# opteroncx/MoePhoto

Hardware: AMD Instinct MI355X
Metric: megapixels/sec (input), 1080p 4x SR (Net4x a4), 256-px tiles with overlap (higher is better)
Workload: dtype fp16; 1 GPU; BASELINE configs[1]: 1 frame(s) 1920x1080 RGB -> 7680x4320, model a4 (Net4x, synthetic weights in zoo format), crop 256 pad 5 align 8 -> 40 tiles/frame, fp16 I/O, fp16 MFMA operands + fp32 accumulate; tiles_per_frame=40, parallelism=single GPU, precision=mixed, exact_blocks=1, input=natural-image-like synthetic frame (tests/golden_defs.natural_image)

## Files before the change

### include/moephoto_amd.h

```cpp
#ifndef MOEPHOTO_AMD_H
#define MOEPHOTO_AMD_H

#include <stddef.h>
#include <stdint.h>

#ifdef __cplusplus
extern "C" {
#endif

#define MOE_ABI_VERSION 4

#define MOE_OK 0
#define MOE_EINVAL (-1)
#define MOE_ENOMEM (-2)
#define MOE_EHIP (-3)
#define MOE_ESTATE (-4)

#define MOE_ARCH_NET2X 0
#define MOE_ARCH_NET3X 1
#define MOE_ARCH_NET4X 2
#define MOE_ARCH_NETDN 3
#define MOE_ARCH_SEDN 4
#define MOE_ARCH_LITE 5

// ... 2 lines not shown
#define MOE_U8 2
#define MOE_U16 3

#define MOE_PREC_FP16 0
#define MOE_PREC_FP16X3 1
#define MOE_PREC_DEBUG_DIRECT 2
#define MOE_PREC_MIXED 3

#define MOE_PREC_AUTO 4

typedef struct moe_net moe_net;
typedef struct moe_plan moe_plan;

const char* moe_last_error(void);
int moe_abi_version(void);
int moe_device_count(void);

int moe_device_info(int device, int64_t info[8]);

int moe_net_create(int arch, int scale, moe_net** out);
void moe_net_destroy(moe_net* net);
int moe_net_scale(const moe_net* net);
int moe_net_num_params(const moe_net* net);
int moe_net_param_info(const moe_net* net, int index, const char** name, int64_t shape[4], int* ndim);
int moe_net_set_param(moe_net* net, const char* name, const float* data, const int64_t* shape, int ndim);
int moe_net_finalize(moe_net* net, int device, int precision);
int moe_net_resolved_precision(const moe_net* net, int precision);
int moe_net_calibrate(moe_net* net, double target, int* blocks, double* err, void* stream);
int moe_net_exact_blocks(const moe_net* net);
int64_t moe_net_workspace_bytes(const moe_net* net, int B, int h, int w);
int64_t moe_net_max_tile_pixels(const moe_net* net);
int moe_net_forward(moe_net* net, const void* x, int x_dtype, int B, int h, int w,
                    int64_t sB, int64_t sH, int64_t sW, const int64_t* x_off,
                    void* y, int y_dtype, const int64_t* y_off, void* stream);
#define MOE_FWD_INPUT_SINCE_PREV 1u
int moe_net_forward_ex(moe_net* net, const void* x, int x_dtype, int B, int h, int w,
                       int64_t sB, int64_t sH, int64_t sW, const int64_t* x_off,
                       void* y, int y_dtype, const int64_t* y_off, void* stream, unsigned flags);
int moe_net_set_profile(moe_net* net, const char* layer_substrings);
int moe_net_get_profile_at(moe_net* net, int index, double* total_ms, int64_t* launches, double* flops);
int moe_net_get_profile(moe_net* net, double* total_ms, int64_t* launches, double* flops);
int moe_net_set_exact_blocks(moe_net* net, int blocks);
int moe_net_set_option(moe_net* net, const char* key, const char* value);
int moe_net_set_debug(moe_net* net, int enable);
int64_t moe_net_debug_tap(moe_net* net, const char* tap, float* host, int64_t capacity, int64_t shape[4], void* stream);

int moe_plan_create(const int64_t shape[3], double ram, double ram_coef, int pad, int scale, int align,
                    int cropsize, moe_plan** out);
void moe_plan_destroy(moe_plan* plan);
int moe_plan_info(const moe_plan* plan, int64_t info[12]);
int moe_plan_tiles(const moe_plan* plan, int32_t* tiles);
int moe_plan_ramp(const moe_plan* plan, float* ramp);
int moe_plan_rows(const moe_plan* plan, int32_t* rows);

int moe_stitch(const moe_plan* plan, int device, const float* tiles_dev, const int64_t* tile_off, int C,
               void* out, int out_dtype, void* stream);
int moe_stitch_dev(const moe_plan* plan, int device, const float* tiles_dev, const int64_t* tile_off_dev, int C,
                   void* out, int out_dtype, void* stream);
int moe_stitch_band(const moe_plan* plan, int device, const float* tiles_dev, const int64_t* tile_off_dev, int C,
                    void* out, int out_dtype, int row0, int row1, int strip, void* stream);
int moe_blend_tile(const void* r, int64_t r_sC, int64_t r_sH, void* canvas, int64_t c_sC, int64_t c_sH, int dtype, int C,
                   int top_sc, int left_sc, int bsc, int rsc, int topT, int leftT, int pad_sc, const void* ramp, void* stream);

typedef struct moe_wire_rec {
    int64_t tile_off;
    int64_t wire_off;
    int32_t C, th, tw;
    int32_t ra0, ra1, rb0, rb1;
    int32_t ca0, ca1, cb0, cb1;
    int32_t reserved;
} moe_wire_rec;
int moe_plan_seams(const moe_plan* plan, int32_t* seams );
int64_t moe_wire_words(const moe_wire_rec* rec);
int moe_wire_pack(const float* tiles_dev, void* wire_dev, const moe_wire_rec* recs_dev, int n, int64_t max_elems, void* stream);
int moe_wire_unpack(float* tiles_dev, const void* wire_dev, const moe_wire_rec* recs_dev, int n, int64_t max_elems, void* stream);

int moe_run_plan(moe_net* net, const moe_plan* plan, const void* img, int img_dtype, int64_t sC, int64_t sH, int64_t sW,
                 void* out, int out_dtype, int max_tiles_per_batch, void* stream);

int moe_run_plan_ex(moe_net* net, const moe_plan* plan, const void* img, int img_dtype, int64_t sC, int64_t sH, int64_t sW,
                    void* out, int out_dtype, int max_tiles_per_batch, float* pool, int shard_index, int shard_count,
                    int do_stitch, void* stream);

int moe_run_plan_frames(moe_net* net, const moe_plan* plan, const void* imgs, int img_dtype, int64_t frame_stride,
                        int64_t sC, int64_t sH, int64_t sW, int n_frames, float* pools, int64_t pool_stride,
                        int owner_index, int owner_count, int max_tiles_per_batch, void* stream);
int moe_run_plan_tiles(moe_net* net, const moe_plan* plan, const void* imgs, int img_dtype, int64_t frame_stride,
                       int64_t sC, int64_t sH, int64_t sW, int n_frames, float* dst, const int64_t* tile_dst,
                       int max_tiles_per_batch, void* stream);
int64_t moe_plan_pool_elems(const moe_plan* plan, int C);
int moe_plan_tile_offsets(const moe_plan* plan, int C, int64_t* off);

int moe_to_float(const void* src, int src_dtype, int bits, int H, int W, int C, void* dst, int dst_dtype, int device, void* stream);
int moe_to_output(const void* src, int src_dtype, int H, int W, int C, int bits, void* dst, int dst_dtype, int device, void* stream);

#define MOE_RESIZE_NEAREST 0
#define MOE_RESIZE_BILINEAR 1
#define MOE_RESIZE_BICUBIC 2
int moe_resize(const void* src, void* dst, int dtype, int C, int H, int W, int h, int w, int mode, int device, void* stream);

#ifdef __cplusplus
}
#endif
#endif
```

### moephoto_amd/_lib.py

```python
import ctypes
import os

HERE = os.path.dirname(os.path.abspath(__file__))
LIB_PATH = os.path.join(HERE, 'libmoephoto_amd.so')

OK, EINVAL, ENOMEM, EHIP, ESTATE = 0, -1, -2, -3, -4
ARCH_NET2X, ARCH_NET3X, ARCH_NET4X, ARCH_NETDN, ARCH_SEDN, ARCH_LITE = range(6)
F32, F16, U8, U16 = range(4)
PREC_FP16, PREC_FP16X3, PREC_DEBUG_DIRECT, PREC_MIXED, PREC_AUTO = range(5)
ABI_VERSION = 4
FWD_INPUT_SINCE_PREV = 1
RESIZE_MODES = {'nearest': 0, 'bilinear': 1, 'bicubic': 2}
PRECISIONS = {'fp16': PREC_FP16, 'fp16x3': PREC_FP16X3, 'debug_direct': PREC_DEBUG_DIRECT, 'mixed': PREC_MIXED}

_lib = None


class EngineError(RuntimeError):
    pass


def lib():
    global _lib
    if _lib is not None:
        return _lib
    if not os.path.exists(LIB_PATH):
        raise EngineError('{} not found: build it with `python -m moephoto_amd.build` (hipcc, gfx950). '
                          'moephoto_amd has no CPU path.'.format(LIB_PATH))
    try:
        import torch
    except ImportError:
        pass
    L = ctypes.CDLL(LIB_PATH)
    c_int, c_i64, c_vp, c_dbl = ctypes.c_int, ctypes.c_int64, ctypes.c_void_p, ctypes.c_double
    P = ctypes.POINTER
    sig = {
        'moe_last_error': (ctypes.c_char_p, []),
        'moe_abi_version': (c_int, []),
        'moe_device_count': (c_int, []),
        'moe_net_create': (c_int, [c_int, c_int, P(c_vp)]),
        'moe_net_destroy': (None, [c_vp]),
        'moe_net_scale': (c_int, [c_vp]),
        'moe_net_num_params': (c_int, [c_vp]),
        'moe_net_param_info': (c_int, [c_vp, c_int, P(ctypes.c_char_p), P(c_i64), P(c_int)]),
        'moe_net_set_param': (c_int, [c_vp, ctypes.c_char_p, c_vp, P(c_i64), c_int]),
        'moe_net_finalize': (c_int, [c_vp, c_int, c_int]),
        'moe_net_resolved_precision': (c_int, [c_vp, c_int]),
        'moe_net_calibrate': (c_int, [c_vp, c_dbl, P(c_int), P(c_dbl), c_vp]),
        'moe_net_exact_blocks': (c_int, [c_vp]),
        'moe_net_workspace_bytes': (c_i64, [c_vp, c_int, c_int, c_int]),
        'moe_net_max_tile_pixels': (c_i64, [c_vp]),
        'moe_net_forward': (c_int, [c_vp, c_vp, c_int, c_int, c_int, c_int, c_i64, c_i64, c_i64, c_vp, c_vp, c_int, c_vp, c_vp]),
        'moe_net_forward_ex': (c_int, [c_vp, c_vp, c_int, c_int, c_int, c_int, c_i64, c_i64, c_i64, c_vp, c_vp, c_int, c_vp, c_vp, ctypes.c_uint]),
        'moe_net_set_profile': (c_int, [c_vp, ctypes.c_char_p]),
        'moe_net_get_profile': (c_int, [c_vp, P(c_dbl), P(c_i64), P(c_dbl)]),
        'moe_net_get_profile_at': (c_int, [c_vp, c_int, P(c_dbl), P(c_i64), P(c_dbl)]),
        'moe_net_set_exact_blocks': (c_int, [c_vp, c_int]),
        'moe_net_set_debug': (c_int, [c_vp, c_int]),
        'moe_net_set_option': (c_int, [c_vp, ctypes.c_char_p, ctypes.c_char_p]),
        'moe_device_info': (c_int, [c_int, P(c_i64)]),
        'moe_blend_tile': (c_int, [c_vp, c_i64, c_i64, c_vp, c_i64, c_i64, c_int, c_int, c_int, c_int, c_int, c_int, c_int, c_int, c_int, c_vp, c_vp]),
        'moe_stitch_dev': (c_int, [c_vp, c_int, c_vp, c_vp, c_int, c_vp, c_int, c_vp]),
        'moe_stitch_band': (c_int, [c_vp, c_int, c_vp, c_vp, c_int, c_vp, c_int, c_int, c_int, c_int, c_vp]),
        'moe_net_debug_tap': (c_i64, [c_vp, ctypes.c_char_p, c_vp, c_i64, P(c_i64), c_vp]),
        'moe_plan_create': (c_int, [P(c_i64), c_dbl, c_dbl, c_int, c_int, c_int, c_int, P(c_vp)]),
        'moe_plan_destroy': (None, [c_vp]),
        'moe_plan_info': (c_int, [c_vp, P(c_i64)]),
        'moe_plan_tiles': (c_int, [c_vp, P(ctypes.c_int32)]),
        'moe_plan_ramp': (c_int, [c_vp, P(ctypes.c_float)]),
        'moe_plan_rows': (c_int, [c_vp, P(ctypes.c_int32)]),
        'moe_plan_seams': (c_int, [c_vp, P(ctypes.c_int32)]),
        'moe_wire_words': (c_i64, [c_vp]),
        'moe_wire_pack': (c_int, [c_vp, c_vp, c_vp, c_int, c_i64, c_vp]),
        'moe_wire_unpack': (c_int, [c_vp, c_vp, c_vp, c_int, c_i64, c_vp]),
        'moe_plan_pool_elems': (c_i64, [c_vp, c_int]),
        'moe_plan_tile_offsets': (c_int, [c_vp, c_int, P(c_i64)]),
        'moe_stitch': (c_int, [c_vp, c_int, c_vp, c_vp, c_int, c_vp, c_int, c_vp]),
        'moe_run_plan': (c_int, [c_vp, c_vp, c_vp, c_int, c_i64, c_i64, c_i64, c_vp, c_int, c_int, c_vp]),
        'moe_run_plan_ex': (c_int, [c_vp, c_vp, c_vp, c_int, c_i64, c_i64, c_i64, c_vp, c_int, c_int, c_vp, c_int, c_int, c_int, c_vp]),
        'moe_run_plan_frames': (c_int, [c_vp, c_vp, c_vp, c_int, c_i64, c_i64, c_i64, c_i64, c_int, c_vp, c_i64, c_int, c_int, c_int, c_vp]),
        'moe_run_plan_tiles': (c_int, [c_vp, c_vp, c_vp, c_int, c_i64, c_i64, c_i64, c_i64, c_int, c_vp, P(c_i64), c_int, c_vp]),
        'moe_to_float': (c_int, [c_vp, c_int, c_int, c_int, c_int, c_int, c_vp, c_int, c_int, c_vp]),
        'moe_to_output': (c_int, [c_vp, c_int, c_int, c_int, c_int, c_int, c_vp, c_int, c_int, c_vp]),
        'moe_resize': (c_int, [c_vp, c_vp, c_int, c_int, c_int, c_int, c_int, c_int, c_int, c_int, c_vp]),
    }
    for name, (res, args) in sig.items():
        fn = getattr(L, name)
        fn.restype, fn.argtypes = res, args
    if L.moe_abi_version() != ABI_VERSION:
        raise EngineError('libmoephoto_amd.so ABI version {} != {}: rebuild it (python -m moephoto_amd.build)'.format(L.moe_abi_version(), ABI_VERSION))
    _lib = L
    return L


EXPORTS = ['moe_last_error', 'moe_abi_version', 'moe_device_count', 'moe_net_create', 'moe_net_destroy', 'moe_net_scale',
           'moe_net_num_params', 'moe_net_param_info', 'moe_net_set_param', 'moe_net_finalize', 'moe_net_resolved_precision', 'moe_net_calibrate', 'moe_net_exact_blocks', 'moe_net_workspace_bytes',
           'moe_net_max_tile_pixels', 'moe_net_forward', 'moe_net_forward_ex', 'moe_net_set_profile', 'moe_net_get_profile', 'moe_net_get_profile_at', 'moe_net_set_exact_blocks', 'moe_net_set_debug', 'moe_net_set_option', 'moe_device_info', 'moe_blend_tile', 'moe_stitch_dev', 'moe_stitch_band', 'moe_net_debug_tap', 'moe_plan_create', 'moe_plan_destroy', 'moe_plan_info',
           'moe_plan_tiles', 'moe_plan_ramp', 'moe_plan_rows', 'moe_plan_seams', 'moe_wire_words', 'moe_wire_pack', 'moe_wire_unpack', 'moe_plan_pool_elems', 'moe_plan_tile_offsets', 'moe_stitch', 'moe_run_plan',
           'moe_run_plan_ex', 'moe_run_plan_frames', 'moe_run_plan_tiles', 'moe_to_float', 'moe_to_output', 'moe_resize']


def check(rc):
    if rc is not None and rc < 0:
        msg = lib().moe_last_error().decode('utf-8', 'replace')
        if rc == ENOMEM:
            raise MemoryError(msg)
        raise EngineError(msg)
    return rc


def device_info(device=0):
    info = (ctypes.c_int64 * 8)()
    check(lib().moe_device_info(int(device), info))
    keys = ('compute_units', 'clock_khz', 'mem_clock_khz', 'mem_bus_bits', 'l2_bytes', 'total_mem_bytes', 'wall_clock_khz', 'lds_bytes_per_cu')
    return dict(zip(keys, [int(v) for v in info]))


def require_device():
    n = lib().moe_device_count()
    if n < 1:
        raise EngineError('no HIP device visible: moephoto_amd runs on MI355X (gfx950) only and has no CPU path')
    return n
```

### moephoto_amd/build.py

```python
import hashlib
import os
import subprocess
import sys

HERE = os.path.dirname(os.path.abspath(__file__))
CSRC = os.path.join(HERE, 'csrc')
SOURCES = ['conv_mfma.hip', 'conv3x3_sp.hip', 'conv3x3_rw.hip', 'conv3x3_ps4.hip', 'conv3x3_ps9.hip', 'arsb32c.hip', 'conv64_x3.hip', 'conv64_q8.hip', 'conv64_sq.hip', 'arsb_sq.hip', 'conv64_s.hip', 'conv1x1.hip', 'conv1x1_f2.hip', 'misc_kernels.hip', 'blend.hip',
           'errors.cpp', 'options.cpp', 'weights.cpp', 'forward.cpp', 'forward_arsb.cpp', 'forward_sedn.cpp', 'forward_lite.cpp', 'calibrate.cpp', 'plan_run.cpp', 'planner.cpp']
HEADERS = ['common.h', 'engine.h', 'net.h', 'rowtile.h', os.path.join('..', '..', 'include', 'moephoto_amd.h')]
LIB = os.path.join(HERE, 'libmoephoto_amd.so')
ARCH = 'gfx950'
EXTRA_FLAGS = {'blend.hip': ['-ffp-contract=off'],
               'arsb32c.hip': ['-fno-slp-vectorize', '-fno-honor-nans', '-mllvm', '-amdgpu-mfma-vgpr-form=1'], 'conv64_x3.hip': ['-fno-slp-vectorize'], 'conv64_q8.hip': ['-fno-slp-vectorize', '-fno-honor-nans', '-mllvm', '-amdgpu-mfma-vgpr-form=1'], 'conv64_sq.hip': ['-fno-slp-vectorize', '-fno-honor-nans', '-mllvm', '-amdgpu-mfma-vgpr-form=1'], 'arsb_sq.hip': ['-fno-slp-vectorize', '-fno-honor-nans', '-mllvm', '-amdgpu-mfma-vgpr-form=1'], 'conv64_s.hip': ['-fno-slp-vectorize', '-fno-honor-nans', '-mllvm', '-amdgpu-mfma-vgpr-form=1'], 'conv1x1.hip': ['-fno-slp-vectorize', '-mllvm', '-amdgpu-mfma-vgpr-form=1'], 'conv1x1_f2.hip': ['-fno-slp-vectorize', '-mllvm', '-amdgpu-mfma-vgpr-form=1'], 'conv3x3_sp.hip': ['-fno-honor-nans'], 'conv3x3_rw.hip': ['-fno-honor-nans', '-fno-slp-vectorize'],
               'conv3x3_ps4.hip': ['-fno-honor-nans', '-fno-slp-vectorize', '-mllvm', '-amdgpu-mfma-vgpr-form=1'],
               'conv3x3_ps9.hip': ['-fno-honor-nans', '-fno-slp-vectorize', '-mllvm', '-amdgpu-mfma-vgpr-form=1']}


def hipcc():
    for c in (os.environ.get('HIPCC'), '/opt/rocm/bin/hipcc', 'hipcc'):
        if c and (os.path.isabs(c) and os.path.exists(c) or not os.path.isabs(c)):
            return c
    return 'hipcc'


def source_digest():
    import hashlib
    h = hashlib.sha256()
    for f in sorted(SOURCES + HEADERS[:-1]) + HEADERS[-1:]:
        h.update(f.encode())
        h.update(open(os.path.join(CSRC, f), 'rb').read())
    return h.hexdigest()


def _compile_cmd(src, extra=()):
    obj = os.path.join(HERE, '_obj', os.path.splitext(src)[0] + '.o')
    cmd = [hipcc(), '--offload-arch=' + ARCH, '-O3', '-std=c++17', '-fPIC', '-x', 'hip', '-c', os.path.join(CSRC, src), '-o', obj]
    cmd += ['-cuid=moe_' + os.path.splitext(src)[0]]
    cmd += EXTRA_FLAGS.get(src, []) + list(extra)
    rel = [c.replace(CSRC, '<csrc>').replace(HERE, '<pkg>') for c in cmd[1:]]
    return cmd, hashlib.sha256('\0'.join(rel).encode()).hexdigest()


def stale():
    if not os.path.exists(LIB):
        return True
    t = os.path.getmtime(LIB)
    for src in SOURCES:
        tag = os.path.join(HERE, '_obj', os.path.splitext(src)[0] + '.o.cmd')
        if not os.path.exists(tag) or open(tag).read().strip() != _compile_cmd(src)[1]:
            return True
    return os.environ.get('MOE_HIPCC_FLAGS') is not None or any(os.path.getmtime(os.path.join(CSRC, f)) > t for f in SOURCES + HEADERS)


def build_lib(force=False, verbose=False):
    if not force and not stale():
        return LIB
    objs = []
    os.makedirs(os.path.join(HERE, '_obj'), exist_ok=True)
    keep = {os.path.splitext(src)[0] + e for src in SOURCES for e in ('.o', '.o.cmd')}
    for old in os.listdir(os.path.join(HERE, '_obj')):
        if old not in keep:
            os.remove(os.path.join(HERE, '_obj', old))
    extra = os.environ.get('MOE_HIPCC_FLAGS', '').split()
    hdr_t = max(os.path.getmtime(os.path.join(CSRC, h)) for h in HEADERS)
    jobs = []
    for src in SOURCES:
        obj = os.path.join(HERE, '_obj', os.path.splitext(src)[0] + '.o')
        objs.append(obj)
        cmd, want = _compile_cmd(src, extra)
        tag = obj + '.cmd'
        have = open(tag).read().strip() if os.path.exists(tag) else ''
        if not force and have == want and os.path.exists(obj) and os.path.getmtime(obj) > max(hdr_t, os.path.getmtime(os.path.join(CSRC, src))):
            continue
        if os.path.exists(tag):
            os.remove(tag)
        if verbose:
            print(' '.join(cmd))
        jobs.append((src, subprocess.Popen(cmd), tag, want))
        running = [j[1] for j in jobs if j[1].poll() is None]
        if len(running) >= max(1, min(8, (os.cpu_count() or 2) // 2)):
            running[0].wait()
    bad = []
    for src, proc, tag, want in jobs:
        if proc.wait() != 0:
            bad.append(src)
        else:
            open(tag, 'w').write(want + '\n')
    if bad:
        raise subprocess.CalledProcessError(1, 'hipcc ' + ' '.join(bad))
    cmd = [hipcc(), '--offload-arch=' + ARCH, '-shared', '-fPIC', '-o', LIB] + objs
    if verbose:
        print(' '.join(cmd))
# ... 24 lines not shown
```

### moephoto_amd/csrc/common.h

```cpp
#pragma once
#include <hip/hip_runtime.h>
#include <stdint.h>

typedef _Float16 half_t;
typedef __attribute__((ext_vector_type(2))) _Float16 half2_t;
typedef __attribute__((ext_vector_type(4))) _Float16 half4_t;
typedef __attribute__((ext_vector_type(8))) _Float16 half8_t;
typedef __attribute__((ext_vector_type(4))) float float4_t;
typedef __attribute__((ext_vector_type(16))) float float16_t;

constexpr int kCB = 64;
constexpr int kTileW = 32;
constexpr int kTileH = 8;
constexpr int kFragBytes = 1024;

struct ConvArgs {
    const half_t* in;
    half_t* out;
    const half_t* res;
    const half_t* wpk;
    const float* bias;
    const float* bias_img;
    const half_t* zero;
    half_t* trash;
// ... 257 lines not shown
    const half_t* in0; const half_t* in1;
    const half_t* w0; const half_t* w1;
    const half_t* in0_lo; const half_t* in1_lo;
    const half_t* w0_lo; const half_t* w1_lo;
    int in1_lo8;
    const void* skip; int skip_dtype;
    const long long* skip_off; long long skip_sB, skip_sH, skip_sW;
    void* y; int y_dtype;
    const long long* y_off;
    int B, H, W, taps;
};
void launch_tail(const TailArgs& a, hipStream_t s);

struct TapSumArgs {
    const float* t0; const float* t1;
    void* y; int y_dtype; const long long* y_off;
    int B, H, W;
    int r;
    int form;
    int vec_ok;
};
void launch_tapsum(const TapSumArgs& a, hipStream_t s);

struct Tail1SumArgs {
    const float* p0; const float* p1;
    int nparts;
    void* y; int y_dtype; const long long* y_off;
    int B, H, W;
    const float* lut; int r; const void* x; const long long* x_off; long long sB, sH, sW;
    int vec_ok;
};
void launch_tail1sum(const Tail1SumArgs& a, hipStream_t s);

void launch_pool_partial(const half_t* in, const half_t* in_lo, float* partial, int B, long long HW, int C, int nslab, hipStream_t s);

struct SednSeArgs {
    const float* partial; int nslab; long long HW;
    const float* w_down;
    const float* w_up;
    const float* trans_pk32;
    half_t* trans_out;
    half_t* trans_out_lo;
    int B, nfrag;
};
void launch_sedn_se(const SednSeArgs& a, hipStream_t s);

struct SednFuseArgs {
    const half_t* x;
    float* partial;
    const float* pooled; int pooled_slabs;
    int pooled_count;
    int nslab, B, H, W;
    const float* w256t;
    const float* w256;
    const float* wt;
    const float* w_down;
    const float* w_up;
    float* gate;
    half_t* weff;
};
void launch_sedn_fuse(const SednFuseArgs& a, hipStream_t s);

struct FrmArgs {
    const float* partial; int nslab; long long HW;
    const float* w0; const float* b0;
    const float* w2; const float* b2;
    const half_t* t; const half_t* x; half_t* out;
    const half_t* t_lo; const half_t* x_lo; half_t* out_lo;
    float* gate;
    int B;
};
void launch_frm(const FrmArgs& a, hipStream_t s);
struct FrmPreArgs {
    const half_t* m; const half_t* m_lo;
    const float* partial; int nslab;
    const float* c2t;
    const float* w0; const float* b0;
    const float* w2; const float* b2;
    float* gate;
    int B, H, W;
};
void launch_frm_pre(const FrmPreArgs& a, hipStream_t s);

struct StitchArgs {
    const float* tiles; const long long* tile_off;
    const int* row_first; const int* row_cnt;
    const int* col_first; const int* col_cnt;
    const int* row_tab; const int* col_tab;
    const float* ramp;
    void* out; int out_dtype;
    int C, out_h, out_w, step_w;
    int row_lo;
    int y0, rows;
};
void launch_stitch(const StitchArgs& a, hipStream_t s);

struct BlendTileArgs {
    const void* r; void* canvas; const void* ramp;
    long long r_sC, r_sH, c_sC, c_sH;
    int C, rh, rw;
    int top_sc, left_sc;
    int r0, c0;
    int lt_h, lt_w;
};
void launch_blend_tile(const BlendTileArgs& a, bool f16, hipStream_t s);

struct WireRec {
    long long tile_off, wire_off;
    int C, th, tw;
    int ra0, ra1, rb0, rb1;
    int ca0, ca1, cb0, cb1;
    int pad_;
};
long long wire_rec_words(const WireRec& r);
void launch_wire(bool pack, float* tiles, unsigned* wire, const WireRec* recs, int n, long long max_elems, hipStream_t s);

void launch_to_float(const void* src, int src_dtype, float inv_or_div, bool divide, int H, int W, int C, void* dst, int dst_dtype, hipStream_t s);
void launch_to_output(const void* src, int src_dtype, int H, int W, int C, float quant, void* dst, int dst_dtype, hipStream_t s);
void launch_resize(const void* src, void* dst, int dtype, int C, int H, int W, int h, int w, int mode, hipStream_t s);
void launch_maxabsdiff(const float* a, const float* b, long long n, unsigned* out, hipStream_t s);
void launch_nhwc_to_nchw_f32(const half_t* in, const half_t* in_lo, float* out, int B, int H, int W, int cs, int C, hipStream_t s);
```

### moephoto_amd/csrc/conv3x3_ps4.hip

```cpp
#include "common.h"
#include "rowtile.h"
#include "../../include/moephoto_amd.h"
#include <algorithm>
#include <type_traits>

#ifndef PS4_FILL
#define PS4_FILL 5
#endif
#ifndef PS4_ZSKIP
#define PS4_ZSKIP 1
#endif
#ifndef PS4_ABL
#define PS4_ABL 0
#endif

namespace {

constexpr int RB = 4;
constexpr int PW = kTileW + 2;
constexpr int ROWB = PW * 128;
constexpr int BLKB = RB * ROWB;
constexpr int NPIECE = BLKB / 1024;
constexpr int TREC = 36 * 128 + 64;
constexpr int TEXP = 36 * 128;
constexpr int TROWS = 16;
constexpr int OFF_T = 2 * BLKB;
constexpr int OFF_BIAS = OFF_T + TROWS * TREC;
constexpr int OFF_TW = OFF_BIAS + 1024;
constexpr int OFF_DUMP = OFF_TW + 8 * 1024;
constexpr int LDS_BYTES = OFF_DUMP + 1024;

typedef unsigned u4_t __attribute__((ext_vector_type(4)));
typedef unsigned u2_t __attribute__((ext_vector_type(2)));
typedef float float2_t __attribute__((ext_vector_type(2)));
typedef const __attribute__((address_space(3))) half8_t* lds_h8_t;

enum OpKind : int { OP_NONE = 0, OP_P, OP_WL, OP_TM, OP_TW, OP_BI, OP_DMA, OP_FA, OP_FR, OP_FS, OP_AR, OP_AS, OP_ST };
struct Op { int kind, a, b, c; };
struct OpList {
    int n = 0;
    Op op[64] = {};
    constexpr void push(int kind, int a = 0, int b = 0, int c = 0) { op[n] = Op{kind, a, b, c}; ++n; }
    constexpr void append(const OpList& o) { for (int i = 0; i < o.n; ++i) { op[n] = o.op[i]; ++n; } }
};
constexpr OpList row_ops(int epi)
{
    OpList r;
    if (epi == 0) {
        for (int s = 0; s < 4; ++s) {
            r.push(OP_P, s >> 1, 4 * (s & 1), 2); r.push(OP_P, s >> 1, 4 * (s & 1) + 2, 2);
            r.push(OP_ST, s >> 1, s & 1);
        }
        return r;
    }
    const bool split = epi == 2;
    int nl = 0;
    auto wl = [&](int frag) { r.push(OP_WL, frag, nl & 1); ++nl; };
    int nt = 0;
    wl(0);
    wl(split ? 4 : 1);
    for (int s = 0; s < 4; ++s) {
        if (split) for (int k = 0; k < 4; ++k) r.push(OP_P, s >> 1, 4 * (s & 1) + k, 1);
        else for (int k = 0; k < 4; k += 2) r.push(OP_P, s >> 1, 4 * (s & 1) + k, 2);
        r.push(OP_TM, nt & 1, 0, nt == 0); ++nt;
        if (split) {
            if (s < 3) wl(s + 1);
            r.push(OP_TM, nt & 1, 1, 0); ++nt;
            if (s < 3) wl(4 + s + 1);
        } else if (s + 2 < 4) wl(s + 2);
    }
    for (int k = 0; k < 5; ++k) r.push(OP_TW, k);
    return r;
}
constexpr OpList extra_ops(int e, bool tail)
{
    OpList r;
    if (!tail) {
        if (e == 0) for (int m = 0; m < 3; ++m) { r.push(OP_DMA, m, 0); r.push(OP_DMA, m, 1); }
        if (e == 1) for (int m = 3; m < 5; ++m) { r.push(OP_DMA, m, 0); r.push(OP_DMA, m, 1); }
        return r;
    }
    if (e == 0) {
        r.push(OP_FA);
        for (int dy = 0; dy < 3; ++dy) { r.push(OP_FR, dy, 0); r.push(OP_FR, dy, 1); r.push(OP_FR, dy, 2); }
// ... 337 lines not shown
                            constexpr int I = decltype(I_)::value;
                            if constexpr (I >= x_lo && I < x_hi) {
                                constexpr Op o = LX.op[I];
                                if constexpr (o.kind != OP_DMA && (PS4_ABL & 2)) return;
                                if constexpr (o.kind == OP_DMA && (PS4_ABL & 64)) return;
                                if constexpr (o.kind == OP_DMA) op_dma(std::integral_constant<int, o.a>{}, std::integral_constant<int, o.b>{});
                                if constexpr (o.kind == OP_FA) op_fa();
                                if constexpr (o.kind == OP_FR) op_fr(std::integral_constant<int, o.a>{}, std::integral_constant<int, o.b>{});
                                if constexpr (o.kind == OP_FS) op_fs();
                                if constexpr (o.kind == OP_AR) op_ar();
                                if constexpr (o.kind == OP_AS) op_as();
                            }
                        };
#define PS4_M(I) runm(std::integral_constant<int, I>{});
                        PS4_M(0) PS4_M(1) PS4_M(2) PS4_M(3) PS4_M(4) PS4_M(5) PS4_M(6) PS4_M(7) PS4_M(8) PS4_M(9) PS4_M(10) PS4_M(11) PS4_M(12) PS4_M(13) PS4_M(14) PS4_M(15)
                        PS4_M(16) PS4_M(17) PS4_M(18) PS4_M(19) PS4_M(20) PS4_M(21) PS4_M(22) PS4_M(23) PS4_M(24) PS4_M(25) PS4_M(26) PS4_M(27) PS4_M(28) PS4_M(29) PS4_M(30) PS4_M(31)
                        PS4_M(32) PS4_M(33) PS4_M(34) PS4_M(35) PS4_M(36) PS4_M(37) PS4_M(38) PS4_M(39) PS4_M(40) PS4_M(41) PS4_M(42) PS4_M(43) PS4_M(44) PS4_M(45) PS4_M(46) PS4_M(47)
#undef PS4_M
#define PS4_X(I) runx(std::integral_constant<int, I>{});
                        PS4_X(0) PS4_X(1) PS4_X(2) PS4_X(3) PS4_X(4) PS4_X(5) PS4_X(6) PS4_X(7) PS4_X(8) PS4_X(9) PS4_X(10) PS4_X(11) PS4_X(12) PS4_X(13) PS4_X(14) PS4_X(15)
#undef PS4_X
                        if (f == 10 && hc == 1 && !(PS4_ABL & 4)) op_bi(std::integral_constant<int, 0>{});
                        if (f == 11 && hc == 1 && !(PS4_ABL & 4)) op_bi(std::integral_constant<int, 1>{});
                    };
                    half(std::integral_constant<int, 0>{});
                    half(std::integral_constant<int, 1>{});
#ifndef PS4_NOPIN
#pragma unroll
                    for (int hc = 0; hc < (ZERO ? 0 : 2); ++hc) {
                        const int h = 2 * f + hc;
                        const int MH = TAIL ? 20 : 10;
                        const int m_lo = h < MH ? h * LM.n / MH : LM.n, m_hi = h < MH ? (h + 1) * LM.n / MH : LM.n;
                        const int ntm = (PS4_ABL & 33) ? 0 : count_kind(LM, m_lo, m_hi, OP_TM);
#pragma unroll
                        for (int i_ = 0; i_ < 3; ++i_) {
                            __builtin_amdgcn_sched_group_barrier(0x008, 1, 0);
                            if (i_ == 0 && hc == 0) __builtin_amdgcn_sched_group_barrier(0x100, 1, 0);
                            __builtin_amdgcn_sched_group_barrier(0x006, PS4_FILL, 0);
                        }
#pragma unroll
                        for (int i_ = 0; i_ < 2; ++i_)
                            if (TAIL && i_ < ntm) { __builtin_amdgcn_sched_group_barrier(0x008, 1, 0); __builtin_amdgcn_sched_group_barrier(0x006, PS4_FILL, 0); }
                    }
#endif
                    __builtin_amdgcn_sched_barrier(0);
                };
#if PS4_ABL
                if constexpr (!LAST) asm volatile("" ::"v"(acc[SL][0]), "v"(acc[SL][1]), "v"(Gt));
#endif
#define PS4_CHUNK(F) chunk(std::integral_constant<int, F>{});
                PS4_CHUNK(0) PS4_CHUNK(1) PS4_CHUNK(2) PS4_CHUNK(3) PS4_CHUNK(4) PS4_CHUNK(5) PS4_CHUNK(6) PS4_CHUNK(7) PS4_CHUNK(8) PS4_CHUNK(9) PS4_CHUNK(10) PS4_CHUNK(11)
#undef PS4_CHUNK
            };
            step(std::integral_constant<int, 0>{});
            step(std::integral_constant<int, 1>{});
            step(std::integral_constant<int, 2>{});
            step(std::integral_constant<int, 3>{});
        };

        typedef std::integral_constant<int, 0> Run;
        typedef std::integral_constant<int, 1> Zero;
        typedef std::integral_constant<int, 2> Last;
        int k = kfirst;
        for (; k + 1 < kz; k += 2) {
            block(k, std::integral_constant<int, 0>{}, Run{});
            block(k + 1, std::integral_constant<int, 1>{}, Run{});
        }
        if (k < kz) { block(k, std::integral_constant<int, 0>{}, Run{}); ++k; }
        if (k < nblk - 1) { block(k, std::integral_constant<int, 0>{}, Zero{}); ++k; }
        if (TAIL) block(k, std::integral_constant<int, 0>{}, Last{});
    }
#endif
}

template <bool VEC>
__global__ __launch_bounds__(256) void tailadd_kernel(TailAddArgs a)
{
    const int nq = a.W >> 3;
    const long long idx = (long long)blockIdx.x * 256 + threadIdx.x;
    if (idx >= (long long)a.B * a.H * nq) return;
    const int xq = (int)(idx % nq);
    const int Y = (int)((idx / nq) % a.H), b = (int)(idx / ((long long)nq * a.H));
    const int X0 = xq * 8;
    const long long po = ((long long)b * a.H + Y) * a.W + X0;
    float v[8];
    {
        const float4 r0 = *(const float4*)(a.p0 + po), r1 = *(const float4*)(a.p0 + po + 4);
        v[0] = r0.x; v[1] = r0.y; v[2] = r0.z; v[3] = r0.w; v[4] = r1.x; v[5] = r1.y; v[6] = r1.z; v[7] = r1.w;
        if (a.p1) {
            const float4 u0 = *(const float4*)(a.p1 + po), u1 = *(const float4*)(a.p1 + po + 4);
            v[0] += u0.x; v[1] += u0.y; v[2] += u0.z; v[3] += u0.w; v[4] += u1.x; v[5] += u1.y; v[6] += u1.z; v[7] += u1.w;
        }
    }
    const int c = X0 >> 6, in = X0 & 63;
    const long long as = (long long)a.B * a.px * a.H;
    if (in == 0 && c >= 1) {
        const long long o = ((long long)b * a.px + (c - 1)) * a.H + Y;
        float t = a.a0[o];
        if (a.a1) t += a.a1[o];
        v[0] += t;
    }
    if (in == 56 && c + 1 < a.px) {
        const long long o = as + ((long long)b * a.px + (c + 1)) * a.H + Y;
        float t = a.a0[o];
        if (a.a1) t += a.a1[o];
        v[7] += t;
    }
    const long long yo = (a.y_off ? a.y_off[b] : (long long)b * a.H * a.W) + (long long)Y * a.W + X0;
    if (a.y_dtype == MOE_F16) {
        if (VEC) {
            half8_t h;
#pragma unroll
            for (int k = 0; k < 8; ++k) h[k] = (half_t)v[k];
            *(half8_t*)((half_t*)a.y + yo) = h;
        } else {
#pragma unroll
            for (int k = 0; k < 8; ++k) ((half_t*)a.y)[yo + k] = (half_t)v[k];
        }
    } else {
        float* yp = (float*)a.y + yo;
        if (VEC) {
            *(float4*)yp = make_float4(v[0], v[1], v[2], v[3]);
            *(float4*)(yp + 4) = make_float4(v[4], v[5], v[6], v[7]);
        } else {
#pragma unroll
            for (int k = 0; k < 8; ++k) yp[k] = v[k];
        }
    }
}

template <int EPI, bool MASK>
hipError_t set_limit()
{
    return hipFuncSetAttribute((const void*)conv3x3_ps4_kernel<EPI, MASK>, hipFuncAttributeMaxDynamicSharedMemorySize, LDS_BYTES);
}

}

hipError_t conv3x3_ps4_init()
{
    hipError_t e;
    if ((e = set_limit<0, true>()) != hipSuccess) return e;
    if ((e = set_limit<1, false>()) != hipSuccess) return e;
    if ((e = set_limit<1, true>()) != hipSuccess) return e;
    if ((e = set_limit<2, false>()) != hipSuccess) return e;
    return set_limit<2, true>();
}

size_t ps4_plane_bytes(int B, int H, int W) { return (size_t)B * H * W * 16; }
size_t ps4_apron_bytes(int B, int H, int W) { return (size_t)2 * B * ((W + kTileW - 1) / kTileW) * 2 * H * 4; }

bool ps4_applicable(int B, int H, int W)
{
    if (H % RB != 0 || W % 4 != 0 || H < RB) return false;
    if ((long long)B * H * W * 128 + (long long)(RB * W + 1) * 128 >= (1ll << 32) - 65536) return false;
    return (long long)B * ((W + kTileW - 1) / kTileW) * (H / RB) < (1ll << 31) / 4;
}

bool ps4_store_applicable(int B, int H, int W, float slope)
{
    return ps4_tail_applicable(B, H, W, slope) && (long long)B * H * W * 512 < (1ll << 32) - 65536;
}

bool launch_conv3x3_ps4(const Ps4Args& a, int max_groups, hipStream_t s)
{
    if (!(a.out ? ps4_store_applicable(a.B, a.H, a.W, a.slope) : ps4_tail_applicable(a.B, a.H, a.W, a.slope))) return false;
    const int px = (a.W + kTileW - 1) / kTileW;
    const long long items = (long long)a.B * px * (a.H / RB);
    const int G = (int)std::min<long long>(items, max_groups);
    const bool ragged = a.W % kTileW != 0;
    if (a.out) {
        if (a.plane) return false;
        conv3x3_ps4_kernel<0, true><<<dim3(G), dim3(256), LDS_BYTES, s>>>(a);
        return true;
    }
    if (a.split) {
        if (ragged) conv3x3_ps4_kernel<2, true><<<dim3(G), dim3(256), LDS_BYTES, s>>>(a);
        else conv3x3_ps4_kernel<2, false><<<dim3(G), dim3(256), LDS_BYTES, s>>>(a);
    } else {
        if (ragged) conv3x3_ps4_kernel<1, true><<<dim3(G), dim3(256), LDS_BYTES, s>>>(a);
        else conv3x3_ps4_kernel<1, false><<<dim3(G), dim3(256), LDS_BYTES, s>>>(a);
    }
    return true;
}

void launch_tailadd(const TailAddArgs& a, hipStream_t s)
{
    const long long n = (long long)a.B * a.H * (a.W / 8);
    if (a.vec_ok) tailadd_kernel<true><<<dim3((unsigned)((n + 255) / 256)), dim3(256), 0, s>>>(a);
    else tailadd_kernel<false><<<dim3((unsigned)((n + 255) / 256)), dim3(256), 0, s>>>(a);
// ... 2 lines not shown
```

### moephoto_amd/csrc/engine.h

```cpp
#pragma once
#include <cstdint>
#include <map>
#include <memory>
#include <string>
#include <utility>
#include <vector>

#include "../../include/moephoto_amd.h"
#include "common.h"

namespace moe {

struct AxisAnchors {
    std::vector<int64_t> start, end, end_sc;
    int64_t clip = 0;
    int step = 1;
};
AxisAnchors get_anchors(int64_t s, int64_t ns, int64_t l, int pad, int align, int sc);

struct TileRect { int top, bottom, left, right, top_t, left_t, bsc, rsc; };

struct PlanDeviceCache {
    int device = -1;
    int C = 0;
    int64_t sC = 0, sH = 0, sW = 0;
    int shard_index = 0, shard_count = 1;
    bool y_mult8 = false;
    std::vector<int> group_first, group_count;
    void* blob = nullptr;
    long long* x_off = nullptr;
    long long* y_off = nullptr;
    long long* tile_off = nullptr;
    int *row_first = nullptr, *row_cnt = nullptr, *col_first = nullptr, *col_cnt = nullptr, *row_tab = nullptr, *col_tab = nullptr;
    float* ramp = nullptr;
    std::vector<std::pair<int, int*>> strip_tabs;
};

struct FramesDeviceCache {
    int device = -1, C = 0, n_frames = 0;
    int64_t sC = 0, sH = 0, sW = 0, frame_stride = 0;
    std::vector<long long> tile_dst;
    bool y_mult8 = false;
    std::vector<int> group_first, group_count;
    void* blob = nullptr;
    long long* x_off = nullptr;
    long long* y_off = nullptr;
};

struct CustomOffsets { int device; std::vector<long long> host; long long* dev; };

struct TileGroup { int th, tw; std::vector<int> tiles; int first_slot; };

struct Plan {
    int C = 0, H = 0, W = 0, pad = 0, sc = 1, align = 8;
    int tile_h = 0, tile_w = 0, pad_sc = 0, out_h = 0, out_w = 0, pad_h_to = 0, pad_w_to = 0;
    AxisAnchors ah, aw;
    std::vector<TileRect> tiles;
    std::vector<float> ramp;
    std::vector<int> row_tab, col_tab, row_first, row_cnt, col_first, col_cnt;
    std::vector<TileGroup> groups;
    std::vector<long long> tile_off;
    size_t pool_elems_per_plane_set = 0;
    mutable std::vector<std::unique_ptr<PlanDeviceCache>> dev;
    mutable std::vector<std::unique_ptr<FramesDeviceCache>> fdev;
    mutable std::vector<CustomOffsets> custom_off;
    mutable float* pool = nullptr;
    mutable size_t pool_elems = 0;
};
int build_plan(Plan& p, const int64_t shape[3], double ram, double ram_coef, int pad, int sc, int align, int cropsize,
               std::string& err);

}
```

### moephoto_amd/csrc/forward.cpp

```cpp
#include "net.h"

using namespace moe;

namespace moe {

const char* kernel_name(ConvKernel k)
{
    static const char* const names[] = {"no kernel", "conv_direct", "conv1x1", "conv_mfma", "conv3x3_sp", "conv3x3_rw", "conv3x3_ps4 (store form)", "conv3x3_sp (hi + lo residual)",
                                        "conv_mfma (three products)", "conv64_x3", "conv64_q8", "conv64_sq", "conv3x3_sp (three launches)", "conv_mfma (fp32 side buffer)"};
    return names[(int)k];
}

static bool fast_layer(const moe_net& n, const ConvLayer& L) { return L.taps == 9 && L.nseg == 1 && !L.per_plane && n.opt.conv_impl == 2; }

ConvForm Fwd::form(const ConvLayer& L, int H, int W) const
{
    ConvForm c;
    c.B = B; c.H = H; c.W = W; c.in_cs = 64 * L.nseg; c.out_cs = L.r > 1 ? 64 : 64 * L.nchunks; c.r = L.r; c.nchunks = L.nchunks;
    c.py = (H + kTileH - 1) / kTileH;
    const long long items = (long long)B * ((W + kTileW - 1) / kTileW) * c.py;
    const int per_xcd = groups / 8;
    int G = per_xcd >= L.nchunks ? 8 * (per_xcd / L.nchunks) : groups / L.nchunks;
    if (G < 1) G = 1;
    if (G > items) G = (int)items;
// ... 243 lines not shown
    best = (size_t)B * (size_t)HW * 64;
    for (int s = 0; s < n.stages; ++s) {
        best = std::max<size_t>(best, (size_t)B * (size_t)HW * rr * rr * 64 * n.r * n.r);
        rr *= n.r;
    }
    return best;
}

int exact_blocks_of(const moe_net& n)
{
    if (n.exact_blocks >= 0) return n.exact_blocks > 6 ? 6 : n.exact_blocks;
    const int env = n.opt.exact_blocks_env;
    if (env >= 0) return env > 6 ? 6 : env;
    if (n.calib_valid && n.calib_blocks >= 0) return n.calib_blocks;
    return default_exact_blocks(n.arch);
}

int default_exact_blocks(int arch)
{
    switch (arch) {
        case MOE_ARCH_NET2X: return 4;
        case MOE_ARCH_NET3X: return 2;
        case MOE_ARCH_NET4X: return 1;
        case MOE_ARCH_NETDN: return 1;
        default: return 0;
    }
}

long long sp_bytes_per_pixel(const moe_net& n)
{
    long long per = 128;
    if (n.arch == MOE_ARCH_SEDN) per = 512;
    if (n.arch == MOE_ARCH_LITE) {
        for (int st = 0; st + 1 < n.stages; ++st) per *= 4;
    }
    if (n.arch == MOE_ARCH_NET2X || n.arch == MOE_ARCH_NET3X || n.arch == MOE_ARCH_NET4X) {
        long long rr = 1;
        for (int st = 0; st < n.stages; ++st) {
            rr *= (long long)n.r * n.r;
            per = std::max(per, st == n.stages - 1 ? 36 * rr : 128 * rr);
        }
    }
    return per;
}

static int run_forward(const moe_net& n, Fwd& f, const FwdIO& io)
{
    const int B = f.B, h = f.h, w = f.w;
    const long long P = (long long)B * h * w;
    f.io = io;
    if (f.x3) {
        f.acc32_elems = acc32_need(n, B, h, w);
        f.acc32 = (float*)f.ar.take(f.acc32_elems * 4);
        f.side16 = (half_t*)f.ar.take(f.acc32_elems * 2 + 4096);
    } else if (f.mixed) {
        f.side16 = (half_t*)f.ar.take((size_t)P * 64 * 2 + 4096);
        bool steep = false;
        for (int i = 1; i <= exact_blocks_of(n); ++i) steep = steep || n.convs[n.conv_index.at("c1_" + std::to_string(i))].slope > 1.f;
        if (steep) { f.acc32_elems = (size_t)P * 64; f.acc32 = (float*)f.ar.take(f.acc32_elems * 4); }
    }
    int rc = MOE_OK;
    switch (n.arch) {
        case MOE_ARCH_SEDN: rc = forward_sedn(n, f); break;
        case MOE_ARCH_LITE: rc = forward_lite(n, f); break;
        default: rc = forward_arsb(n, f);
    }
    return rc ? rc : f.rc;
}

static Fwd make_fwd(const moe_net& n, const FwdCtx& ctx, NetRuntime* rt, hipStream_t s, int B, int h, int w, Arena ar)
{
    Fwd f{n, ctx, rt, s, B, h, w, ar, ctx.groups, n.precision == MOE_PREC_FP16X3, n.precision == MOE_PREC_DEBUG_DIRECT};
    f.mixed = n.precision == MOE_PREC_MIXED;
    return f;
}

static size_t workspace_need(const moe_net& n, const FwdCtx& ctx, int B, int h, int w)
{
    Fwd f = make_fwd(n, ctx, nullptr, nullptr, B, h, w, Arena{});
    run_forward(n, f, FwdIO{});
    return f.ar.off + 4096;
}

static bool plan_matches(const Fwd& f, size_t planned)
{
    if (f.ar.overflow) return false;
    return f.skips_planned_work ? f.ar.off <= planned : f.ar.off == planned;
}

static int forward_dev_chunk(moe_net& n, const FwdIO& io, int B, int h, int w, hipStream_t s, bool y_off_mult8, const FwdCtx& ctx);

static void build_lite_lut_on_device(moe_net& n, hipStream_t s, const FwdCtx& ctx)
{
    const int r = n.scale;
    std::vector<unsigned short> pat(65536);
    for (int i = 0; i < 65536; ++i) pat[(size_t)i] = (unsigned short)i;
    half_t* in = nullptr;
    float* scratch = nullptr;
    int rc = MOE_ENOMEM;
    if (hipMalloc((void**)&in, 65536 * 2) == hipSuccess && hipMalloc((void**)&n.lut, (size_t)65536 * r * r * 4) == hipSuccess && hipMalloc((void**)&scratch, (size_t)65536 * r * r * 4) == hipSuccess &&
        hipMemcpyAsync(in, pat.data(), 65536 * 2, hipMemcpyHostToDevice, s) == hipSuccess && hipStreamSynchronize(s) == hipSuccess) {
        FwdCtx capture = ctx;
        capture.lut_capture = n.lut;
        rc = forward_dev_chunk(n, FwdIO{in, MOE_F16, 65536, 256, 1, nullptr, scratch, MOE_F32, nullptr}, 1, 256, 256, s, true, capture);
        (void)hipStreamSynchronize(s);
    }
    if (in) (void)hipFree(in);
    if (scratch) (void)hipFree(scratch);
    if (rc != MOE_OK) { (void)hipGetLastError(); drop_lut(n); }
    n.lut_state = rc == MOE_OK ? 1 : -1;
}

static void build_lite_lut(moe_net& n, hipStream_t s, const FwdCtx& ctx)
{
    n.lut_state = -1;
    if (n.arch != MOE_ARCH_LITE || !n.opt.lite_lut || n.debug || !n.opt.fuse_tail || n.precision == MOE_PREC_DEBUG_DIRECT) return;
    hipStreamCaptureStatus cs = hipStreamCaptureStatusNone;
    if (hipStreamIsCapturing(s, &cs) != hipSuccess || cs != hipStreamCaptureStatusNone) { (void)hipGetLastError(); n.lut_state = 0; return; }
    int cur = -1;
    if (hipGetDevice(&cur) != hipSuccess || (cur != n.device && hipSetDevice(n.device) != hipSuccess)) { (void)hipGetLastError(); n.lut_state = 0; return; }
    build_lite_lut_on_device(n, s, ctx);
    if (cur != n.device) (void)hipSetDevice(cur);
}

int forward_dev(moe_net& n, const FwdIO& io, int B, int h, int w, hipStream_t s, bool y_off_mult8, const FwdCtx& ctx)
{
    if (!n.finalized) return fail(MOE_ESTATE, "moe_net_forward: net is not finalized (load_state_dict + to(device) first)");
    if (B < 1 || h < 1 || w < 1) return fail(MOE_EINVAL, "moe_net_forward: bad shape B=%d h=%d w=%d", B, h, w);
    if ((io.x_dtype != MOE_F32 && io.x_dtype != MOE_F16) || (io.y_dtype != MOE_F32 && io.y_dtype != MOE_F16))
        return fail(MOE_EINVAL, "moe_net_forward: x/y dtype must be MOE_F32 or MOE_F16");
    const long long bmax = kSpRange / (sp_bytes_per_pixel(n) * (long long)h * w);
    if (bmax < 1)
        return fail(MOE_ENOMEM, "a %dx%d tile exceeds the convolution kernels' addressing range (%lld pixels per plane at most for this net): use a smaller cropsize",
                    h, w, kSpRange / sp_bytes_per_pixel(n));
    if (n.arch == MOE_ARCH_LITE && io.x_dtype == MOE_F16 && n.lut_state == 0 && n.opt.lite_lut) build_lite_lut(n, s, ctx);
    if (B <= bmax) return forward_dev_chunk(n, io, B, h, w, s, y_off_mult8, ctx);
    const size_t xe = io.x_dtype == MOE_F32 ? 4 : 2, ye = io.y_dtype == MOE_F32 ? 4 : 2;
    const long long yplane = (long long)h * n.scale * w * n.scale;
    for (int b0 = 0; b0 < B; b0 += (int)bmax) {
        const int cnt = (int)std::min<long long>(bmax, B - b0);
        FwdIO c = io;
        if (io.x_off) c.x_off += b0; else c.x = (const char*)io.x + (size_t)b0 * io.sB * xe;
        if (io.y_off) c.y_off += b0; else c.y = (char*)io.y + (size_t)b0 * yplane * ye;
        const bool al = y_off_mult8 && (io.y_off || ((size_t)b0 * yplane * ye) % 16 == 0);
        if (int rc = forward_dev_chunk(n, c, cnt, h, w, s, al, ctx)) return rc;
    }
    return MOE_OK;
}

static int forward_dev_chunk(moe_net& n, const FwdIO& io, int B, int h, int w, hipStream_t s, bool y_off_mult8, const FwdCtx& ctx)
{
    int cur = -1;
    HIP_TRY(hipGetDevice(&cur));
    if (cur != n.device) HIP_TRY(hipSetDevice(n.device));
    const size_t need = workspace_need(n, ctx, B, h, w);
    StreamSet& set = *ctx.set;
    if (need > set.ws_bytes) {
        if (set.ws) { HIP_TRY(hipStreamSynchronize(s)); HIP_TRY(hipFree(set.ws)); set.ws = nullptr; set.ws_bytes = 0; }
        hipError_t e = hipMalloc((void**)&set.ws, need);
        if (e != hipSuccess) { (void)hipGetLastError(); return fail(MOE_ENOMEM, "workspace of %zu bytes for %d planes of %dx%d does not fit", need, B, h, w); }
        set.ws_bytes = need;
    }
    const size_t planned = need - 4096;
    Fwd f = make_fwd(n, ctx, &n.rt, s, B, h, w, Arena{set.ws, 0, planned});
    f.y_vec = y_off_mult8 && ((uintptr_t)io.y % 16 == 0);
    int rc = run_forward(n, f, io);
    if (rc) return rc;
    if (!plan_matches(f, planned))
        return fail(MOE_EINVAL, "internal error: the launching pass took %zu bytes of workspace%s, the planning pass %zu (%d planes of %dx%d)", f.ar.off,
                    f.ar.overflow ? " (beyond the plan: the launches behind that point were not issued)" : "", planned, B, h, w);
    hipError_t e = hipGetLastError();
    if (e != hipSuccess) return fail(MOE_EHIP, "kernel launch failed: %s", hipGetErrorString(e));
    return MOE_OK;
}

void free_set(StreamSet& set)
{
    if (set.side) { (void)hipStreamSynchronize(set.side); (void)hipStreamDestroy(set.side); }
    for (hipEvent_t e : {set.ev_fork, set.ev_join}) if (e) (void)hipEventDestroy(e);
    if (set.ws) (void)hipFree(set.ws);
    set = StreamSet{};
}

void free_records(NetRuntime& rt)
{
    for (auto& ev : rt.prof_ev) { (void)hipEventDestroy(ev.e0); (void)hipEventDestroy(ev.e1); }
    for (auto& sl : rt.off_ring) {
        if (sl.host) (void)hipHostFree(sl.host);
        if (sl.dev) (void)hipFree(sl.dev);
        if (sl.done) (void)hipEventDestroy(sl.done);
    }
    for (auto& t : rt.taps) if (t.second.dev) (void)hipFree(t.second.dev);
    rt = NetRuntime{};
}

void pipe_destroy(moe_net& n)
{
    for (auto& ps : n.pipe) {
        if (ps.main) { (void)hipStreamSynchronize(ps.main); (void)hipStreamDestroy(ps.main); }
        for (hipEvent_t e : {ps.entry, ps.done}) if (e) (void)hipEventDestroy(e);
        free_set(ps);
        ps = PipeSet{};
    }
    n.pipe_prev_valid = false;
    n.pipe_last_stream = nullptr;
}

static bool overlap_eligible(const moe_net& n, int B, int h, int w)
{
    const bool sr = n.arch == MOE_ARCH_NET2X || n.arch == MOE_ARCH_NET3X || n.arch == MOE_ARCH_NET4X;
    return sr && n.finalized && n.opt.overlap_calls && !n.debug && n.opt.conv_impl == 2 && (n.precision == MOE_PREC_MIXED || n.precision == MOE_PREC_FP16) &&
           (long long)B * h * w <= 4ll * 65536 && n.prof_keys.empty() && n.opt.repeat_key.empty();
}

static int forward_pipelined(moe_net* n, const void* x, int x_dtype, int B, int h, int w, int64_t sB, int64_t sH, int64_t sW, void* y, int y_dtype, hipStream_t s, unsigned flags)
{
    HIP_TRY(hipSetDevice(n->device));
    PipeSet& ps = n->pipe[n->pipe_next];
    PipeSet& prev = n->pipe[n->pipe_next ^ 1];
// ... 153 lines not shown
```

### moephoto_amd/csrc/forward_arsb.cpp

```cpp
#include "net.h"

using namespace moe;

namespace {

const ConvLayer* last_up(const moe_net& n, int br)
{
    const auto it = n.conv_index.find(std::string(br == 0 ? "convt_R1" : "u") + ".up" + std::to_string(n.stages - 1));
    return it == n.conv_index.end() ? nullptr : &n.convs[it->second];
}

bool can_fuse_tail(const moe_net& n, const Fwd& f)
{
    const int B = f.B, h = f.h, w = f.w;
    if (!n.opt.fuse_tail || f.x3 || f.direct || n.debug || n.opt.conv_impl != 2 || n.stages < 1) return false;
    if (!(n.arch == MOE_ARCH_NET2X || n.arch == MOE_ARCH_NET3X || n.arch == MOE_ARCH_NET4X)) return false;
    if (sp_bytes_per_pixel(n) * B * h * w > kSpRange) return false;
    int hl = h, wl = w;
    for (int st = 0; st + 1 < n.stages; ++st) { hl *= n.r; wl *= n.r; }
    for (int br = 0; br < 2; ++br) {
        const ConvLayer* L = last_up(n, br);
        if (!L) return false;
        ConvForm c = f.form(*L, hl, wl);
        c.tail = true;
        if (!conv3x3_sp_applicable(c)) return false;
    }
    return true;
}

struct ArsbRun {
    const moe_net& n;
    Fwd& f;
    const int B, h, w;
    bool mixed = false;
    int nx = 0;
    Act A, Bb, Cc;
    bool chain8 = false;
    half_t* lo16x = nullptr;
    bool sr = false, fuse = false, ps4 = false, ps9 = false;
    int H = 0, W = 0;
    Act fin[2];
    float* tp[2] = {nullptr, nullptr};
    float* ps_plane[2] = {nullptr, nullptr};
    float* ps_apron[2] = {nullptr, nullptr};

    void plan_tail_form();
    template <typename Args, typename Launch>
    int ps_stage(int br, const std::string& key, const Act& cur, size_t plane_bytes, size_t apron_bytes, const char* name, Launch launch);
    int run_branch(int br, Act cur);
    int trunk_conv(const std::string& key, const Act& in, const Act& out, const Act* res, bool exact);
    int run_trunk();
    template <typename Args, typename Launch> void tail_add(Launch launch);
    int branch_sum();
    int run();
};

void ArsbRun::plan_tail_form()
{
    sr = n.arch != MOE_ARCH_NETDN;
    fuse = sr && can_fuse_tail(n, f);
    if (sr) {
        int hl = h, wl = w;
        for (int st = 0; st + 1 < n.stages; ++st) { hl *= n.r; wl *= n.r; }
        bool ok = fuse && n.opt.tail_form == 1;
        bool ps4_ok = true;
        bool ps9_ok = true;
        for (int br = 0; br < 2; ++br) {
            const ConvLayer* L = last_up(n, br);
            if (ok) {
                ConvForm c = f.form(*L, hl, wl);
                c.tail = true; c.tail_form = 1;
                ok = conv3x3_rw_applicable(c);
            }
            ps4_ok = ps4_ok && L && ps4_tail_applicable(B, hl, wl, L->slope);
            ps9_ok = ps9_ok && L && ps9_tail_applicable(B, hl, wl, L->slope);
        }
        f.tail_form = ok ? 1 : 0;
        ps4 = ok && n.opt.up_impl == 1 && ps4_ok && (2 * wl) % 8 == 0;
        ps9 = fuse && n.opt.up_impl == 1 && n.r == 3 && f.groups >= 3 && ps9_ok;
    }
}

template <typename Args, typename Launch>
int ArsbRun::ps_stage(int br, const std::string& key, const Act& cur, size_t plane_bytes, size_t apron_bytes, const char* name, Launch launch)
{
    ps_plane[br] = (float*)f.ar.take(plane_bytes + 4096);
    ps_apron[br] = (float*)f.ar.take(apron_bytes + 4096);
    if (!f.dry()) {
        const ConvLayer& L = n.convs[n.conv_index.at(key)];
        Args q{};
        q.in = cur.hi; q.wpk = f.blob<half_t>(L.w_hi); q.bias = L.has_bias ? f.blob<float>(L.bias) : f.small<float>("zero_bias");
        q.tail_w = f.small<half_t>(br == 0 ? "tail_r.frag" : "tail_u.frag");
        q.plane = ps_plane[br]; q.apron = ps_apron[br]; q.slope = L.slope; q.B = B; q.H = H; q.W = W;
        q.split = (f.mixed && f.tail_split_for(key)) ? 1 : 0;
        const int rec = f.prof_begin(key, 2.0 * (double)B * H * W * L.cout * L.cin * L.taps);
        bool done = false;
        for (int rep = f.repeats(key); rep > 0; --rep) done = launch(q, f.groups, f.s);
        f.prof_end(rec);
        if (!done) return fail(MOE_EINVAL, "fused tail kernel (%s) rejected layer %s", name, key.c_str());
    }
    H *= n.r; W *= n.r;
    return (int)MOE_OK;
}

int ArsbRun::run_branch(int br, Act cur)
{
    if (f.mixed) { cur.drop_lo(); cur.lo8 = false; }
    H = h; W = w;
    for (int st = 0; st < n.stages; ++st) {
        const std::string key = std::string(br == 0 ? "convt_R1" : "u") + ".up" + std::to_string(st);
        if (ps4 && st == n.stages - 1) {
            if (int rc = ps_stage<Ps4Args>(br, key, cur, ps4_plane_bytes(B, H, W), ps4_apron_bytes(B, H, W), "ps4", launch_conv3x3_ps4)) return rc;
            continue;
        }
        if (ps9 && st == n.stages - 1) {
            if (int rc = ps_stage<Ps9Args>(br, key, cur, ps9_plane_bytes(B, H, W), ps9_apron_bytes(B, H, W), "ps9", launch_conv3x3_ps9)) return rc;
            continue;
        }
        if (fuse && st == n.stages - 1) {
            tp[br] = (float*)f.ar.take(f.tail_form == 1 ? (size_t)tailsum_layout(B, H, W).total * 4 + 4096 : (size_t)9 * B * H * n.r * W * n.r * 4 + 4096);
            ConvExtra tail;
            tail.fuse_tail = true; tail.tail_w = f.small<half_t>(br == 0 ? "tail_r.frag" : "tail_u.frag"); tail.tplanes = tp[br];
            if (!f.conv(key, cur, Act{}, nullptr, H, W, tail))
                return fail(MOE_EINVAL, "fused tail kernel rejected layer %s", key.c_str());
            H *= n.r; W *= n.r;
            continue;
        }
        Act nxt = f.act((long long)B * H * n.r * W * n.r);
        f.conv(key, cur, nxt, nullptr, H, W);
        H *= n.r; W *= n.r;
        f.tap(std::string(br == 0 ? "r" : "u") + ".up" + std::to_string(st), nxt, H, W, 64, 64);
        cur = nxt;
    }
    fin[br] = cur;
    return (int)MOE_OK;
}

int ArsbRun::trunk_conv(const std::string& key, const Act& in, const Act& out, const Act* res, bool exact)
{
    ConvExtra e;
    e.exact = exact;
    if (!f.conv(key, in, out, res, h, w, e))
        return fail(MOE_EINVAL, "layer %s: %d planes of %dx%d exceed the conv kernel's addressing range (use smaller tiles)", key.c_str(), B, h, w);
    return (int)MOE_OK;
}

int ArsbRun::run_trunk()
{
    if (int rc = trunk_conv("input2", A, Bb, nullptr, mixed)) return rc;
    f.tap("input2", Bb, h, w, 64, n.C);
    const bool arsb_fuse = n.opt.arsb_fuse && !f.x3 && !f.direct && n.opt.conv_impl == 2;
    hipStream_t s = f.s;
    Act cur = Bb, oth = Cc;
    for (int i = 1; i <= 6; ++i) {
        const bool ex = mixed && i <= nx;
        const std::string k1 = "c1_" + std::to_string(i), k2 = "c2_" + std::to_string(i);
        const ConvLayer& L1 = n.convs[n.conv_index.at(k1)];
        const ConvLayer& L2 = n.convs[n.conv_index.at(k2)];
        const bool trunk64 = L1.w_arsb != 0;
        const int cin = (L1.cin == 48 && L2.cin == 48 && n.opt.k48) ? 48 : 64;
        if (arsb_fuse && !ex && (!mixed || (cur.has_lo && oth.has_lo)) && trunk64 && arsb32c_applicable(B, h, w, L1.slope, mixed, mixed, cin)) {
            if (!f.dry()) {
                ArsbArgs q{};
                q.x_hi = cur.hi; q.x_lo = mixed ? cur.lo : nullptr; q.y_hi = oth.hi; q.y_lo = mixed ? oth.lo : nullptr;
                q.w1 = f.blob<half_t>(L1.w_hi); q.w2 = f.blob<half_t>(L2.w_hi); q.zero = f.small<half_t>("zero");
                q.slope = L1.slope; q.B = B; q.H = h; q.W = w; q.cin = cin;
                q.drop_lo = (mixed && i == 6 && n.arch != MOE_ARCH_NETDN && !n.debug) ? 1 : 0;
                const bool trace = n.opt.arsb_trace;
                const size_t tb = 8 * 16 * 4 * 40 * 8;
                if (trace && i == 3 && hipMalloc((void**)&q.trace, tb) == hipSuccess) (void)hipMemsetAsync(q.trace, 0, tb, s);
                const int rec = f.prof_begin("arsb" + std::to_string(i), 2.0 * 2.0 * (double)B * h * w * L1.cout * L1.cin * 9);
                bool done = false;
                for (int rep = f.repeats("arsb" + std::to_string(i)); rep > 0; --rep) done = launch_arsb32c(q, f.groups, s);
                f.prof_end(rec);
                if (q.trace) {
                    std::vector<unsigned long long> host(tb / 8);
                    (void)hipStreamSynchronize(s);
                    (void)hipMemcpy(host.data(), q.trace, tb, hipMemcpyDeviceToHost);
                    if (FILE* fp = fopen("/tmp/arsb_trace.bin", "wb")) { fwrite(host.data(), 1, tb, fp); fclose(fp); }
                    (void)hipFree(q.trace);
                }
                if (!done) return fail(MOE_EINVAL, "internal error: arsb32c rejected layer %s its predicate took", k1.c_str());
            }
            std::swap(cur, oth); cur.lo8 = oth.lo8 = false; f.tap("arsb" + std::to_string(i), cur, h, w, 64, n.C);
            continue;
        }
        if (ex && chain8 && n.opt.exact_fuse && n.opt.q8_impl == 1 && cur.lo8 && cur.has_lo && oth.has_lo && L1.wq_hi8 && L2.wq_hi8 && !L1.has_bias && !L2.has_bias && L2.slope == 1.f &&
            arsb_sq_applicable(B, h, w, L1.slope)) {
            if (!f.dry()) {
                ArsbSqArgs q{};
                q.x_hi = cur.hi; q.x_lo8 = (const unsigned char*)cur.lo; q.y_hi = oth.hi; q.y_lo = oth.lo;
                q.w16[0] = f.blob<half_t>(L1.w_hi); q.wh8[0] = f.blob<unsigned char>(L1.wq_hi8); q.wl8[0] = f.blob<unsigned char>(L1.wq_lo8);
                q.w16[1] = f.blob<half_t>(L2.w_hi); q.wh8[1] = f.blob<unsigned char>(L2.wq_hi8); q.wl8[1] = f.blob<unsigned char>(L2.wq_lo8);
                q.slope = L1.slope; q.B = B; q.H = h; q.W = w; q.out8 = i < nx;
                const int rec = f.prof_begin("xpair" + std::to_string(i), 2.0 * 2.0 * 3.0 * (double)B * h * w * L1.cout * L1.cin * 9);
                const bool done = launch_arsb_sq(q, f.groups, s);
                f.prof_end(rec);
                if (!done) return fail(MOE_EINVAL, "internal error: arsb_sq rejected layer %s its predicate took", k1.c_str());
            }
            std::swap(cur, oth);
            cur.lo8 = i < nx;
            oth.lo8 = false;
            f.tap("arsb" + std::to_string(i), cur, h, w, 64, n.C);
            continue;
        }
        Act m = oth;
        if (mixed && !ex) m.drop_lo();
        m.lo8 = ex && chain8;
        Act bin = cur;
        if (mixed && !ex) bin.drop_lo();
        if (int rc = trunk_conv(k1, bin, m, nullptr, ex)) return rc;
        const Act resid = cur;
        if (ex && chain8 && i == nx) { cur.lo = lo16x ? lo16x : A.lo; cur.lo8 = false; }
        if (int rc = trunk_conv(k2, m, cur, &resid, ex)) return rc;
        f.tap("arsb" + std::to_string(i), cur, h, w, 64, n.C);
    }
    Bb = cur;
    return (int)MOE_OK;
}

template <typename Args, typename Launch>
void ArsbRun::tail_add(Launch launch)
{
    if (f.dry()) return;
    Args t{};
    t.p0 = ps_plane[0]; t.p1 = ps_plane[1]; t.a0 = ps_apron[0]; t.a1 = ps_apron[1];
    t.y = f.io.y; t.y_dtype = f.io.y_dtype; t.y_off = f.io.y_off; t.B = B; t.H = H; t.W = W; t.px = (W / n.r + kTileW - 1) / kTileW;
    t.vec_ok = f.y_vec;
    const int rec = f.prof_begin("tailadd", 0.0);
    f.gate();
    launch(t, f.s);
    f.prof_end(rec);
}

int ArsbRun::branch_sum()
{
    if (ps4) { tail_add<TailAddArgs>(launch_tailadd); return MOE_OK; }
    if (ps9) { tail_add<TailAdd3Args>(launch_tailadd3); return MOE_OK; }
    if (fuse) {
        if (!f.dry()) {
            TapSumArgs t{};
            t.t0 = tp[0]; t.t1 = tp[1]; t.y = f.io.y; t.y_dtype = f.io.y_dtype; t.y_off = f.io.y_off; t.B = B; t.H = H; t.W = W; t.r = n.r;
            t.form = f.tail_form;
            t.vec_ok = n.r == 2 && f.y_vec && W % 8 == 0;
            f.gate();
            launch_tapsum(t, f.s);
        }
        return MOE_OK;
    }
    f.tail(&fin[0], &fin[1], H, W, false);
    return MOE_OK;
}

int ArsbRun::run()
{
    const long long P = (long long)B * h * w;
    hipStream_t s = f.s;
    mixed = f.mixed;
    nx = mixed ? exact_blocks_of(n) : 0;
    A = f.act(P, 64, mixed); Bb = f.act(P, 64, mixed); Cc = f.act(P, 64, mixed);
    if (mixed && n.opt.conv_impl != 2)
        return fail(MOE_EINVAL, "precision 'mixed' runs on the fast 3x3 kernels only: conv_impl=v1 (MOE_CONV_IMPL=v1) is a debugging switch for 'fp16' / 'fp16x3'");
    const bool dn = n.arch == MOE_ARCH_NETDN;
    chain8 = mixed && f.use_q8() && n.opt.lo8 && !n.debug && !f.direct && nx >= 1 && A.has_lo && Bb.has_lo && Cc.has_lo;
    if (dn && (int)n.scalars.at("tail_taps") != 9) chain8 = false;
    for (int i = 0; chain8 && i <= nx; ++i)
        for (int j = (i == 0 ? 2 : 1); chain8 && j <= 2; ++j)
            chain8 = f.q8_capable(n.convs[n.conv_index.at(i == 0 ? std::string("input2") : "c" + std::to_string(j) + "_" + std::to_string(i))]);
    lo16x = (dn && chain8) ? (half_t*)f.ar.take((size_t)P * 64 * 2 + 2048) : nullptr;
    A.lo8 = Bb.lo8 = chain8;
    f.stem(A);
    f.tap("stem", A, h, w, 64, n.C);
    plan_tail_form();
    const bool forked = sr && f.ctx.fork && !n.debug && !f.direct && !f.x3 && n.opt.conv_impl == 2 && (long long)B * h * w <= 4ll * 65536;
    struct ForkGuard {
        StreamSet* set; hipStream_t s; bool armed = false;
        ~ForkGuard()
        {
            if (!armed) return;
            if (hipEventRecord(set->ev_join, set->side) != hipSuccess || hipStreamWaitEvent(s, set->ev_join, 0) != hipSuccess) (void)hipStreamSynchronize(set->side);
        }
    } fork_guard{f.ctx.set, s};
    const int all = f.groups;
    int g_side = 0;
    if (forked && all >= 32) {
        g_side = n.opt.branch_groups > 0 ? n.opt.branch_groups : (n.stages >= 2 ? 5 * all / 16 : 3 * all / 16);
        g_side = std::max(8, std::min(g_side, all - 8) / 8 * 8);
    }
    if (forked) {
        if (g_side) f.groups = g_side;
        if (!f.dry()) {
            StreamSet& set = *f.ctx.set;
            if (!set.side) {
                HIP_TRY(hipStreamCreateWithFlags(&set.side, hipStreamNonBlocking));
                HIP_TRY(hipEventCreateWithFlags(&set.ev_fork, hipEventDisableTiming));
                HIP_TRY(hipEventCreateWithFlags(&set.ev_join, hipEventDisableTiming));
            }
            HIP_TRY(hipEventRecord(set.ev_fork, s));
            HIP_TRY(hipStreamWaitEvent(set.side, set.ev_fork, 0));
            f.s = set.side;
            fork_guard.armed = true;
        }
        const int rc = run_branch(1, A);
        if (g_side) f.groups = all - g_side;
        if (!f.dry()) {
            f.s = s;
            if (!rc) HIP_TRY(hipEventRecord(f.ctx.set->ev_join, f.ctx.set->side));
        }
        if (rc) return rc;
    }
    if (int rc = run_trunk()) return rc;
    if (n.arch == MOE_ARCH_NETDN) { f.tail(&Bb, &A, h, w, false); return MOE_OK; }
    if (mixed) { A.drop_lo(); Bb.drop_lo(); A.lo8 = Bb.lo8 = false; }
    if (!forked) { if (int rc = run_branch(0, Bb)) return rc; if (int rc = run_branch(1, A)) return rc; }
    else {
        if (int rc = run_branch(0, Bb)) return rc;
        if (!f.dry()) { HIP_TRY(hipStreamWaitEvent(s, f.ctx.set->ev_join, 0)); fork_guard.armed = false; }
        f.groups = all;
    }
    return branch_sum();
}

}

int moe::forward_arsb(const moe_net& n, Fwd& f)
{
    ArsbRun r{n, f, f.B, f.h, f.w};
    return r.run();
}
```

### moephoto_amd/csrc/misc_kernels.hip

```cpp
#include "common.h"
#include <algorithm>
#include <cstdlib>
#include <cstring>
#include "../../include/moephoto_amd.h"

namespace {

__device__ __forceinline__ float prelu(float v, float slope) { return v >= 0.f ? v : v * slope; }

template <typename T>
__device__ __forceinline__ float ld1(const void* p, long long i) { return (float)((const T*)p)[i]; }

template <typename TIN, int TAPS>
__global__ __launch_bounds__(256) void stem_kernel(StemArgs a)
{
    __shared__ float w[TAPS * 64];
    for (int i = threadIdx.x; i < TAPS * 64; i += 256) w[i] = a.w[i];
    __syncthreads();
    if (a.out_lo8) asm volatile("s_setreg_imm32_b32 hwreg(HW_REG_MODE, 23, 1), 1\n\ts_nop 3" ::: "memory");
    constexpr int PX = 8;
    const int nq = (a.W + PX - 1) / PX;
    const long long idx = (long long)blockIdx.x * 256 + threadIdx.x;
    const long long q = idx >> 3;
    if (q >= (long long)a.B * a.H * nq) return;
    const int cg = (int)(idx & 7) * 8;
    const int x0 = (int)(q % nq) * PX;
    const long long t = q / nq;
    const int y = (int)(t % a.H);
    const int b = (int)(t / a.H);
    const TIN* xp = (const TIN*)a.x + (a.x_off ? a.x_off[b] : (long long)b * a.sB);
    constexpr int KD = (TAPS == 9) ? 3 : 1, PAD = (TAPS == 9) ? 1 : 0;
    float wr[TAPS][8];
#pragma unroll
    for (int k = 0; k < TAPS; ++k) {
        const float4 w0 = *(const float4*)(w + k * 64 + cg), w1 = *(const float4*)(w + k * 64 + cg + 4);
        wr[k][0] = w0.x; wr[k][1] = w0.y; wr[k][2] = w0.z; wr[k][3] = w0.w;
        wr[k][4] = w1.x; wr[k][5] = w1.y; wr[k][6] = w1.z; wr[k][7] = w1.w;
    }
    float v[KD][PX + 2 * PAD];
#pragma unroll
    for (int dy = 0; dy < KD; ++dy) {
        const int yy = y + dy - PAD;
        const bool rok = yy >= 0 && yy < a.H;
        const TIN* rp = xp + (long long)yy * a.sH;
#pragma unroll
        for (int c = 0; c < PX + 2 * PAD; ++c) {
            const int xx = x0 + c - PAD;
            v[dy][c] = (rok && xx >= 0 && xx < a.W) ? (float)rp[(long long)xx * a.sW] : 0.f;
        }
    }
#pragma unroll
    for (int e4 = 0; e4 < PX; ++e4) {
        float acc[8] = {0, 0, 0, 0, 0, 0, 0, 0};
#pragma unroll
        for (int dy = 0; dy < KD; ++dy)
#pragma unroll
            for (int dx = 0; dx < KD; ++dx)
#pragma unroll
                for (int e = 0; e < 8; ++e) acc[e] += v[dy][e4 + dx] * wr[dy * KD + dx][e];
        if (x0 + e4 >= a.W) continue;
        const long long p = ((long long)b * a.H + y) * a.W + x0 + e4;
        half8_t o;
#pragma unroll
        for (int e = 0; e < 8; ++e) o[e] = (half_t)prelu(acc[e], a.slope);
        *(half8_t*)(a.out + p * 64 + cg) = o;
        if (a.out_lo) {
            half8_t l;
#pragma unroll
            for (int e = 0; e < 8; ++e) l[e] = (half_t)((prelu(acc[e], a.slope) - (float)o[e]) * 2048.f);
            if (!a.out_lo8) *(half8_t*)(a.out_lo + p * 64 + cg) = l;
            else {
                typedef unsigned u4v __attribute__((ext_vector_type(4)));
                const u4v lw = __builtin_bit_cast(u4v, l);
                unsigned p0, p1;
                const float quarter = 4.0f;
                asm volatile("v_cvt_scalef32_pk_fp8_f16 %0, %2, %6\n\t"
                             "v_cvt_scalef32_pk_fp8_f16 %1, %4, %6\n\t"
                             "v_cvt_scalef32_pk_fp8_f16 %0, %3, %6 op_sel:[0,0,1]\n\t"
                             "v_cvt_scalef32_pk_fp8_f16 %1, %5, %6 op_sel:[0,0,1]\n\t"
                             "s_nop 0"
                             : "=&v"(p0), "=&v"(p1) : "v"(lw[0]), "v"(lw[1]), "v"(lw[2]), "v"(lw[3]), "v"(quarter));
                *(uint2*)((unsigned char*)a.out_lo + p * 64 + cg) = make_uint2(p0, p1);
            }
// ... 821 lines not shown
        if (c == 0) sums[0][ch] = (red[0][ch] + red[1][ch]) + (red[2][ch] + red[3][ch]);
    }
    __syncthreads();
    for (int k = t; k < 576; k += 256) {
        const int tap = k >> 6, ci = k & 63, dy = tap / 3, dx = tap % 3;
        float v = sums[0][ci];
        if (dy == 0) v -= sums[2][ci];
        if (dy == 2) v -= sums[1][ci];
        if (dx == 0) v -= sums[4][ci];
        if (dx == 2) v -= sums[3][ci];
        if (dy == 0 && dx == 0) v += corner[3][ci];
        if (dy == 0 && dx == 2) v += corner[2][ci];
        if (dy == 2 && dx == 0) v += corner[1][ci];
        if (dy == 2 && dx == 2) v += corner[0][ci];
        sh[k] = v;
    }
    __syncthreads();
    {
        const int q = t >> 6, co = t & 63;
        float m0 = 0.f, m1 = 0.f;
#pragma unroll 8
        for (int k = q * 144; k < q * 144 + 144; k += 2) {
            m0 += a.c2t[(k + 0) * 64 + co] * sh[k + 0];
            m1 += a.c2t[(k + 1) * 64 + co] * sh[k + 1];
        }
        red[q][co] = m0 + m1;
    }
    __syncthreads();
    if (t < 64) mean[t] = ((red[0][t] + red[1][t]) + (red[2][t] + red[3][t])) / (float)HW;
    __syncthreads();
    if (t < 3) {
        float h = a.b0[t];
        for (int c = 0; c < 64; ++c) h += a.w0[t * 64 + c] * mean[c];
        hid[t] = h > 0.f ? h : 0.f;
    }
    __syncthreads();
    if (t < 64) {
        float u = a.b2[t];
#pragma unroll
        for (int k = 0; k < 3; ++k) u += a.w2[t * 3 + k] * hid[k];
        const float g = fmaxf(1.f / (1.f + __expf(-u)), 1e-12f);
        a.gate[b * 64 + t] = g;
        a.gate[((long long)a.B + b) * 64 + t] = 1.f / g;
    }
}

__global__ __launch_bounds__(256) void frm_apply_kernel(FrmArgs a)
{
    const long long idx = (long long)blockIdx.x * 256 + threadIdx.x;
    const long long total = (long long)a.B * a.HW * 8;
    if (idx >= total) return;
    const int cg = (int)(idx & 7) * 8;
    const int b = (int)((idx >> 3) / a.HW);
    const float* g = a.gate + b * 64 + cg;
    const half8_t tv = *(const half8_t*)(a.t + idx * 8);
    const half8_t xv = *(const half8_t*)(a.x + idx * 8);
    float v[8];
#pragma unroll
    for (int e = 0; e < 8; ++e) v[e] = (float)tv[e];
    if (a.t_lo) {
        const half8_t tl = *(const half8_t*)(a.t_lo + idx * 8);
#pragma unroll
        for (int e = 0; e < 8; ++e) v[e] += (float)tl[e] * 0.00048828125f;
    }
#pragma unroll
    for (int e = 0; e < 8; ++e) v[e] = v[e] * g[e] + (float)xv[e];
    if (a.x_lo) {
        const half8_t xl = *(const half8_t*)(a.x_lo + idx * 8);
#pragma unroll
        for (int e = 0; e < 8; ++e) v[e] += (float)xl[e] * 0.00048828125f;
    }
    half8_t o;
#pragma unroll
    for (int e = 0; e < 8; ++e) o[e] = (half_t)v[e];
    *(half8_t*)(a.out + idx * 8) = o;
    if (a.out_lo) {
        half8_t l;
#pragma unroll
        for (int e = 0; e < 8; ++e) l[e] = (half_t)((v[e] - (float)o[e]) * 2048.f);
        *(half8_t*)(a.out_lo + idx * 8) = l;
    }
}

__device__ __forceinline__ float stitch_pixel(const StitchArgs& a, int X, int Y, int c)
{
    const int i0 = a.row_first[Y], ni = a.row_cnt[Y];
    const int j0 = a.col_first[X], nj = a.col_cnt[X];
    float cur = 0.f;
    for (int i = max(i0, a.row_lo); i < i0 + ni; ++i) {
        const int fy = a.row_tab[i * 4 + 0], sy = a.row_tab[i * 4 + 1], oy = a.row_tab[i * 4 + 2], eh = a.row_tab[i * 4 + 3];
        for (int j = j0; j < j0 + nj; ++j) {
            const int fx = a.col_tab[j * 4 + 0], sx = a.col_tab[j * 4 + 1], ox = a.col_tab[j * 4 + 2], ew = a.col_tab[j * 4 + 3];
            const float r = a.tiles[a.tile_off[i * a.step_w + j] + ((long long)c * eh + (Y - oy)) * ew + (X - ox)];
            float v1 = r;
            if (Y < sy) v1 = cur + a.ramp[Y - fy] * (r - cur);
            float v = v1;
            if (X < sx) v = cur + a.ramp[X - fx] * (v1 - cur);
            cur = v;
        }
    }
    return cur;
}

__global__ __launch_bounds__(256) void stitch_kernel(StitchArgs a)
{
    const int X = blockIdx.x * 256 + threadIdx.x;
    const int Y = blockIdx.y + a.y0, c = blockIdx.z;
    if (X >= a.out_w) return;
    const float cur = stitch_pixel(a, X, Y, c);
    const long long o = ((long long)c * a.rows + (Y - a.y0)) * a.out_w + X;
    if (a.out_dtype == MOE_F16) ((half_t*)a.out)[o] = (half_t)cur;
    else ((float*)a.out)[o] = cur;
}

__global__ __launch_bounds__(256) void stitch4_kernel(StitchArgs a)
{
    const int X0 = (blockIdx.x * 256 + threadIdx.x) * 4;
    const int Y = blockIdx.y + a.y0, c = blockIdx.z;
    if (X0 >= a.out_w) return;
    float v[4];
    const int i0 = a.row_first[Y], j0 = a.col_first[X0];
    bool fast = a.row_cnt[Y] == 1 && a.col_cnt[X0] == 1 && a.col_cnt[X0 + 3] == 1 && a.col_first[X0 + 3] == j0;
    if (fast) {
        const int sy = a.row_tab[i0 * 4 + 1], oy = a.row_tab[i0 * 4 + 2], eh = a.row_tab[i0 * 4 + 3];
        const int sx = a.col_tab[j0 * 4 + 1], ox = a.col_tab[j0 * 4 + 2], ew = a.col_tab[j0 * 4 + 3];
        const long long o = a.tile_off[i0 * a.step_w + j0] + ((long long)c * eh + (Y - oy)) * ew + (X0 - ox);
        fast = Y >= sy && X0 >= sx && (o & 3) == 0;
        if (fast) {
            const float4 q = *(const float4*)(a.tiles + o);
            v[0] = q.x; v[1] = q.y; v[2] = q.z; v[3] = q.w;
        }
    }
    if (!fast) {
#pragma unroll
        for (int e = 0; e < 4; ++e) v[e] = stitch_pixel(a, X0 + e, Y, c);
    }
    const long long o = ((long long)c * a.rows + (Y - a.y0)) * a.out_w + X0;
    if (a.out_dtype == MOE_F16) {
        half4_t h;
#pragma unroll
        for (int e = 0; e < 4; ++e) h[e] = (half_t)v[e];
        *(half4_t*)((half_t*)a.out + o) = h;
    } else {
        *(float4*)((float*)a.out + o) = make_float4(v[0], v[1], v[2], v[3]);
    }
}

template <int R>
__global__ __launch_bounds__(256) void stitch8r_kernel(StitchArgs a)
{
    __shared__ int s_col[64 * 4];
    __shared__ int s_seam[256];
    __shared__ int s_nseam;
    const int Y0 = blockIdx.y * R + a.y0, c = blockIdx.z;
    const int yend = a.y0 + a.rows;
    const int nsw = a.step_w;
    for (int t = threadIdx.x; t < nsw * 4; t += 256) s_col[t] = a.col_tab[t];
    if (threadIdx.x == 0) s_nseam = 0;
    __syncthreads();
    const int X0 = (blockIdx.x * 256 + threadIdx.x) * 8;
    if (X0 < a.out_w) {
        const int j0 = a.col_first[X0], j7 = a.col_first[X0 + 7];
        bool colfast = a.col_cnt[X0] == 1 && a.col_cnt[X0 + 7] == 1 && j0 == j7;
        const int sx = s_col[j0 * 4 + 1], ox = s_col[j0 * 4 + 2], ew = s_col[j0 * 4 + 3];
        colfast = colfast && X0 >= sx;
        if (!colfast) s_seam[atomicAdd(&s_nseam, 1)] = threadIdx.x;
        else {
            float v[R][8];
#pragma unroll
            for (int r = 0; r < R; ++r) {
                const int Y = min(Y0 + r, yend - 1);
                const int i0 = a.row_first[Y], ni = a.row_cnt[Y];
                float cur[8] = {0.f, 0.f, 0.f, 0.f, 0.f, 0.f, 0.f, 0.f};
                for (int i = max(i0, a.row_lo); i < i0 + ni; ++i) {
                    const int fy = a.row_tab[i * 4 + 0], sy = a.row_tab[i * 4 + 1], oy = a.row_tab[i * 4 + 2], eh = a.row_tab[i * 4 + 3];
                    const long long o = a.tile_off[i * nsw + j0] + ((long long)c * eh + (Y - oy)) * ew + (X0 - ox);
                    float q[8];
                    if ((o & 3) == 0) {
                        const float4 q0 = *(const float4*)(a.tiles + o), q1 = *(const float4*)(a.tiles + o + 4);
                        q[0] = q0.x; q[1] = q0.y; q[2] = q0.z; q[3] = q0.w; q[4] = q1.x; q[5] = q1.y; q[6] = q1.z; q[7] = q1.w;
                    } else {
#pragma unroll
                        for (int e = 0; e < 8; ++e) q[e] = a.tiles[o + e];
                    }
                    if (Y < sy) {
                        const float wgt = a.ramp[Y - fy];
#pragma unroll
                        for (int e = 0; e < 8; ++e) cur[e] = cur[e] + wgt * (q[e] - cur[e]);
                    } else {
#pragma unroll
                        for (int e = 0; e < 8; ++e) cur[e] = q[e];
                    }
                }
#pragma unroll
                for (int e = 0; e < 8; ++e) v[r][e] = cur[e];
            }
#pragma unroll
            for (int r = 0; r < R; ++r) {
                if (Y0 + r >= yend) break;
                const long long o = ((long long)c * a.rows + (Y0 + r - a.y0)) * a.out_w + X0;
                if (a.out_dtype == MOE_F16) {
                    half8_t h;
#pragma unroll
                    for (int e = 0; e < 8; ++e) h[e] = (half_t)v[r][e];
                    *(half8_t*)((half_t*)a.out + o) = h;
                } else {
                    *(float4*)((float*)a.out + o) = make_float4(v[r][0], v[r][1], v[r][2], v[r][3]);
                    *(float4*)((float*)a.out + o + 4) = make_float4(v[r][4], v[r][5], v[r][6], v[r][7]);
                }
            }
        }
    }
    __syncthreads();
    const int total = s_nseam * 8 * R;
    for (int t = threadIdx.x; t < total; t += 256) {
        const int gidx = t / (8 * R), rem = t - gidx * 8 * R;
        const int r = rem >> 3, e = rem & 7;
        const int X = (blockIdx.x * 256 + s_seam[gidx]) * 8 + e, Y = Y0 + r;
        if (Y >= yend) continue;
        const float cur = stitch_pixel(a, X, Y, c);
        const long long o = ((long long)c * a.rows + (Y - a.y0)) * a.out_w + X;
        if (a.out_dtype == MOE_F16) ((half_t*)a.out)[o] = (half_t)cur;
        else ((float*)a.out)[o] = cur;
    }
}

template <typename TS, typename TD>
__global__ void to_float_kernel(const TS* src, TD* dst, int H, int W, int C, float d, bool divide)
{
    const long long idx = (long long)blockIdx.x * 256 + threadIdx.x;
    const long long n = (long long)H * W * C;
    if (idx >= n) return;
    const int c = (int)(idx % C);
    const long long p = idx / C;
    const float v = (float)src[idx];
    dst[(long long)c * H * W + p] = (TD)(divide ? v / d : v * d);
}

template <typename TS, typename TD>
__global__ void to_output_kernel(const TS* src, TD* dst, int H, int W, int C, float quant)
{
    const long long idx = (long long)blockIdx.x * 256 + threadIdx.x;
    const long long n = (long long)H * W * C;
    if (idx >= n) return;
    const int c = (int)(idx % C);
    const long long p = idx / C;
    float v = (float)src[(long long)c * H * W + p] * quant;
    v = fminf(fmaxf(v, 0.f), quant - 1.f);
    if (!(v == v)) v = 0.f;
    dst[idx] = (TD)(int)v;
}

template <typename T, int N> struct alignas(sizeof(T) * 8 >= 16 ? 16 : 8) VecN { T e[N]; };

template <typename TS, typename TD>
__global__ __launch_bounds__(256) void to_float3_kernel(const TS* __restrict__ src, TD* __restrict__ dst, long long HW, float d, bool divide)
{
    const long long p0 = ((long long)blockIdx.x * 256 + threadIdx.x) * 8;
    if (p0 >= HW) return;
    const VecN<TS, 24> in = *(const VecN<TS, 24>*)(src + p0 * 3);
#pragma unroll
    for (int c = 0; c < 3; ++c) {
        VecN<TD, 8> o;
#pragma unroll
        for (int e = 0; e < 8; ++e) {
            const float v = (float)in.e[e * 3 + c];
            o.e[e] = (TD)(divide ? v / d : v * d);
        }
        *(VecN<TD, 8>*)(dst + c * HW + p0) = o;
    }
}

template <typename TS, typename TD>
__global__ __launch_bounds__(256) void to_output3_kernel(const TS* __restrict__ src, TD* __restrict__ dst, long long HW, float quant)
{
    const long long p0 = ((long long)blockIdx.x * 256 + threadIdx.x) * 8;
    if (p0 >= HW) return;
    VecN<TD, 24> o;
#pragma unroll
    for (int c = 0; c < 3; ++c) {
        const VecN<TS, 8> in = *(const VecN<TS, 8>*)(src + c * HW + p0);
#pragma unroll
        for (int e = 0; e < 8; ++e) {
            float v = (float)in.e[e] * quant;
            v = fminf(fmaxf(v, 0.f), quant - 1.f);
            if (!(v == v)) v = 0.f;
            o.e[e * 3 + c] = (TD)(int)v;
        }
    }
    *(VecN<TD, 24>*)(dst + p0 * 3) = o;
}

__global__ void nhwc_to_nchw_kernel(const half_t* in, const half_t* in_lo, float* out, int B, int H, int W, int cs, int C)
{
    const long long idx = (long long)blockIdx.x * 256 + threadIdx.x;
    const long long n = (long long)B * C * H * W;
    if (idx >= n) return;
    const int x = (int)(idx % W);
    long long t = idx / W;
    const int y = (int)(t % H); t /= H;
    const int c = (int)(t % C);
    const int b = (int)(t / C);
    const long long o = ((long long)(b * H + y) * W + x) * cs + c;
    float v = (float)in[o];
    if (in_lo) v += (float)in_lo[o] * 0.00048828125f;
    out[idx] = v;
}

// ... 5 lines not shown
    const int blocks = (int)((n + 255) / 256);
    if (a.taps == 9) {
        if (a.x_dtype == MOE_F16) hipLaunchKernelGGL((stem_kernel<half_t, 9>), dim3(blocks), dim3(256), 0, s, a);
        else hipLaunchKernelGGL((stem_kernel<float, 9>), dim3(blocks), dim3(256), 0, s, a);
    } else {
        if (a.x_dtype == MOE_F16) hipLaunchKernelGGL((stem_kernel<half_t, 1>), dim3(blocks), dim3(256), 0, s, a);
        else hipLaunchKernelGGL((stem_kernel<float, 1>), dim3(blocks), dim3(256), 0, s, a);
    }
}

void launch_tail(const TailArgs& a, hipStream_t s)
{
    static const bool old9 = [] { const char* e = getenv("MOE_TAIL_V1"); return e && !strcmp(e, "1"); }();
    const int blocks = ((a.W + 31) / 32) * ((a.H + 7) / 8) * a.B;
    if (a.taps == 9 && (!old9 || a.in1_lo8)) {
        const dim3 g(((a.W + 29) / 30) * ((a.H + 7) / 8) * a.B);
        if (a.in0_lo && a.in1_lo8) hipLaunchKernelGGL(tail3_kernel<2>, g, dim3(256), 0, s, a);
        else if (a.in0_lo) hipLaunchKernelGGL(tail3_kernel<1>, g, dim3(256), 0, s, a);
        else hipLaunchKernelGGL(tail3_kernel<0>, g, dim3(256), 0, s, a);
    }
    else if (a.taps == 9) hipLaunchKernelGGL((tail_kernel<9>), dim3(blocks), dim3(256), 0, s, a);
    else hipLaunchKernelGGL((tail_kernel<1>), dim3(blocks), dim3(256), 0, s, a);
}

void launch_tapsum(const TapSumArgs& a, hipStream_t s)
{
    if (a.form == 1) {
        const long long n = (long long)a.B * a.H * (a.W / 8);
        if (a.vec_ok) tapsum4_kernel<true><<<dim3((unsigned)((n + 255) / 256)), dim3(256), 0, s>>>(a);
        else tapsum4_kernel<false><<<dim3((unsigned)((n + 255) / 256)), dim3(256), 0, s>>>(a);
        return;
    }
    const dim3 grid((a.W + 255) / 256, a.H, a.B);
    if (a.r == 3) tapsum_kernel<3><<<grid, dim3(256), 0, s>>>(a);
    else if (a.vec_ok) {
        const long long n = (long long)a.B * a.H * (a.W / 8);
        tapsum2_kernel<<<dim3((unsigned)((n + 255) / 256)), dim3(256), 0, s>>>(a);
    } else tapsum_kernel<2><<<grid, dim3(256), 0, s>>>(a);
}

void launch_tail1sum(const Tail1SumArgs& a, hipStream_t s)
{
    if (a.lut && !a.p1 && a.nparts == 1 && a.vec_ok && a.W % 4 == 0 && (a.r == 2 || a.r == 4 || a.r == 8) && ((uintptr_t)a.p0 & 15) == 0) {
        const long long nq = (long long)a.B * a.H * (a.W / 4);
        hipLaunchKernelGGL(tail1sum_lut4_kernel, dim3((unsigned)((nq + 255) / 256)), dim3(256), 0, s, a);
        return;
    }
    const long long n = (long long)a.B * a.H * a.W;
    hipLaunchKernelGGL(tail1sum_kernel, dim3((unsigned)((n + 255) / 256)), dim3(256), 0, s, a);
}

void launch_pool_partial(const half_t* in, const half_t* in_lo, float* partial, int B, long long HW, int C, int nslab, hipStream_t s)
{
    hipLaunchKernelGGL(pool_partial_kernel, dim3(nslab, B), dim3(256), 0, s, in, in_lo, partial, HW, C, nslab);
}

void launch_sedn_se(const SednSeArgs& a, hipStream_t s)
{
    hipLaunchKernelGGL(sedn_se_kernel, dim3(a.B, kSeSplit), dim3(256), 0, s, a);
}

void launch_sedn_fuse(const SednFuseArgs& a, hipStream_t s)
{
    if (!a.pooled) hipLaunchKernelGGL(sedn_xsum_kernel, dim3(a.nslab, a.B), dim3(256), 0, s, a);
    hipLaunchKernelGGL(sedn_fmean_kernel, dim3(a.B, kMeanSplit), dim3(256), 0, s, a);
    hipLaunchKernelGGL(sedn_weff_kernel, dim3(9, a.B), dim3(256), 0, s, a);
}

void launch_frm(const FrmArgs& a, hipStream_t s)
{
    hipLaunchKernelGGL(frm_gate_kernel, dim3(a.B), dim3(256), 0, s, a);
    const long long total = (long long)a.B * a.HW * 8;
    hipLaunchKernelGGL(frm_apply_kernel, dim3((unsigned)((total + 255) / 256)), dim3(256), 0, s, a);
}

void launch_frm_pre(const FrmPreArgs& a, hipStream_t s)
{
    hipLaunchKernelGGL(frm_pre_kernel, dim3(a.B), dim3(256), 0, s, a);
}

void launch_stitch(const StitchArgs& a, hipStream_t s)
{
    if (a.rows <= 0) return;
    if (a.out_w % 8 == 0 && a.step_w <= 64 && ((uintptr_t)a.out & 15) == 0) hipLaunchKernelGGL(stitch8r_kernel<4>, dim3((a.out_w / 8 + 255) / 256, (a.rows + 3) / 4, a.C), dim3(256), 0, s, a);
    else if (a.out_w % 4 == 0 && ((uintptr_t)a.out & 15) == 0) hipLaunchKernelGGL(stitch4_kernel, dim3((a.out_w / 4 + 255) / 256, a.rows, a.C), dim3(256), 0, s, a);
    else hipLaunchKernelGGL(stitch_kernel, dim3((a.out_w + 255) / 256, a.rows, a.C), dim3(256), 0, s, a);
}

__device__ __forceinline__ int wire_slot(int v, int a0, int a1, int b0, int b1)
{
    return (v >= a0 && v < a1) ? v - a0 : (v >= b0 && v < b1) ? (a1 - a0) + v - b0 : -1;
}

template <bool PACK>
__global__ __launch_bounds__(256) void wire_kernel(float* __restrict__ tiles, unsigned* __restrict__ wire, const WireRec* __restrict__ recs)
{
    const WireRec r = recs[blockIdx.y];
    const int nR = (r.ra1 - r.ra0) + (r.rb1 - r.rb0), nC = (r.ca1 - r.ca0) + (r.cb1 - r.cb0);
    const bool raw = nR >= r.th;
    const long long plane = (long long)r.th * r.tw, n = plane * r.C;
    float* t = tiles + r.tile_off;
    unsigned* w = wire + r.wire_off;
    const long long hw = raw ? 0 : (n + 1) / 2;
    half_t* h16 = (half_t*)w;
    float* rows = (float*)(w + hw);
    float* cols = rows + (long long)r.C * nR * r.tw;
    for (long long e = ((long long)blockIdx.x * 256 + threadIdx.x) * 2; e < n; e += (long long)gridDim.x * 512) {
#pragma unroll
        for (int u = 0; u < 2; ++u) {
            const long long q = e + u;
            if (q >= n) break;
            const int c = (int)(q / plane);
            const int rem = (int)(q - c * plane);
            const int y = rem / r.tw, x = rem - y * r.tw;
            const int ry = wire_slot(y, r.ra0, r.ra1, r.rb0, r.rb1);
            const int cx = ry >= 0 ? -1 : wire_slot(x, r.ca0, r.ca1, r.cb0, r.cb1);
            if (PACK) {
                const float v = t[q];
                if (!raw) h16[q] = (half_t)v;
                if (ry >= 0) rows[((long long)c * nR + ry) * r.tw + x] = v;
                else if (cx >= 0) cols[((long long)c * r.th + y) * nC + cx] = v;
            } else {
                t[q] = ry >= 0 ? rows[((long long)c * nR + ry) * r.tw + x] : cx >= 0 ? cols[((long long)c * r.th + y) * nC + cx] : (float)h16[q];
            }
        }
    }
}

long long wire_rec_words(const WireRec& r)
{
    const long long nR = (r.ra1 - r.ra0) + (r.rb1 - r.rb0), nC = (r.ca1 - r.ca0) + (r.cb1 - r.cb0);
    const long long n = (long long)r.C * r.th * r.tw;
    if (nR >= r.th) return n;
    return (n + 1) / 2 + (long long)r.C * nR * r.tw + (long long)r.C * r.th * nC;
}

void launch_wire(bool pack, float* tiles, unsigned* wire, const WireRec* recs, int n, long long max_elems, hipStream_t s)
{
    if (n <= 0) return;
    const unsigned gx = (unsigned)std::min<long long>(std::max<long long>((max_elems + 2047) / 2048, 1), 4096);
    if (pack) hipLaunchKernelGGL(wire_kernel<true>, dim3(gx, n), dim3(256), 0, s, tiles, wire, recs);
    else hipLaunchKernelGGL(wire_kernel<false>, dim3(gx, n), dim3(256), 0, s, tiles, wire, recs);
}

void launch_to_float(const void* src, int src_dtype, float d, bool divide, int H, int W, int C, void* dst, int dst_dtype, hipStream_t s)
{
    const long long n = (long long)H * W * C, HW = (long long)H * W;
    const dim3 blk(256);
    if (C == 3 && HW % 8 == 0 && (((uintptr_t)src | (uintptr_t)dst) & 15) == 0) {
        const dim3 g3((unsigned)((HW / 8 + 255) / 256));
        if (src_dtype == MOE_U8) {
            if (dst_dtype == MOE_F16) hipLaunchKernelGGL((to_float3_kernel<uint8_t, half_t>), g3, blk, 0, s, (const uint8_t*)src, (half_t*)dst, HW, d, divide);
            else hipLaunchKernelGGL((to_float3_kernel<uint8_t, float>), g3, blk, 0, s, (const uint8_t*)src, (float*)dst, HW, d, divide);
        } else {
            if (dst_dtype == MOE_F16) hipLaunchKernelGGL((to_float3_kernel<uint16_t, half_t>), g3, blk, 0, s, (const uint16_t*)src, (half_t*)dst, HW, d, divide);
            else hipLaunchKernelGGL((to_float3_kernel<uint16_t, float>), g3, blk, 0, s, (const uint16_t*)src, (float*)dst, HW, d, divide);
        }
        return;
    }
    const dim3 grid((unsigned)((n + 255) / 256));
    if (src_dtype == MOE_U8) {
        if (dst_dtype == MOE_F16) hipLaunchKernelGGL((to_float_kernel<uint8_t, half_t>), grid, blk, 0, s, (const uint8_t*)src, (half_t*)dst, H, W, C, d, divide);
        else hipLaunchKernelGGL((to_float_kernel<uint8_t, float>), grid, blk, 0, s, (const uint8_t*)src, (float*)dst, H, W, C, d, divide);
    } else {
        if (dst_dtype == MOE_F16) hipLaunchKernelGGL((to_float_kernel<uint16_t, half_t>), grid, blk, 0, s, (const uint16_t*)src, (half_t*)dst, H, W, C, d, divide);
        else hipLaunchKernelGGL((to_float_kernel<uint16_t, float>), grid, blk, 0, s, (const uint16_t*)src, (float*)dst, H, W, C, d, divide);
// ... 120 lines not shown
```

### moephoto_amd/csrc/net.h

```cpp
#pragma once
#include "engine.h"

#include <algorithm>
#include <cmath>
#include <cstdarg>
#include <cstdio>
#include <cstdlib>
#include <cstring>

namespace moe {

int fail(int code, const char* fmt, ...);

#define HIP_TRY(expr)                                                                                    \
    do {                                                                                                 \
        hipError_t e_ = (expr);                                                                          \
        if (e_ != hipSuccess) return fail(e_ == hipErrorOutOfMemory ? MOE_ENOMEM : MOE_EHIP, "%s: %s", #expr, hipGetErrorString(e_)); \
    } while (0)

struct Param {
    std::string name;
    std::vector<int64_t> shape;
    std::vector<float> data;
    bool set = false;
// ... 64 lines not shown
    int calib_log = 0;
    int auto_calibrate = 1;
    int exact_blocks_env = -1;
    int tiles_per_batch = 0;
    int max_groups = 0;
    int dbg = 0;
    std::string trace_key = "convt_R1.up1";
    bool arsb_trace = false;
    std::string repeat_key;
    int repeat_n = 1;


    bool set(const std::string& key, const char* v);
    void from_env();
};

struct StreamSet { char* ws = nullptr; size_t ws_bytes = 0; hipStream_t side = nullptr; hipEvent_t ev_fork = nullptr, ev_join = nullptr; };
struct PipeSet : StreamSet { hipStream_t main = nullptr; hipEvent_t entry = nullptr, done = nullptr; };

struct NetRuntime {
    struct ProfRec { hipEvent_t e0 = nullptr, e1 = nullptr; int key = 0; double flops = 0; };
    std::vector<ProfRec> prof_ev;
    size_t prof_used = 0;
    struct Tap { float* dev = nullptr; int64_t shape[4] = {0, 0, 0, 0}; };
    std::map<std::string, Tap> taps;
    struct OffSlot { long long* host = nullptr; long long* dev = nullptr; size_t cap = 0; hipEvent_t done = nullptr; bool used = false; };
    OffSlot off_ring[4];
    int off_next = 0;
};

}

struct moe_net {
    int arch = 0, scale = 1;
    moe::NetOptions opt;
    int C = 64;
    int stages = 1, r = 2;
    std::vector<moe::Param> params;
    std::map<std::string, int> index;
    bool finalized = false;
    int device = -1, precision = MOE_PREC_FP16;
    int exact_blocks = -1;
    bool calib_valid = false;
    float* lut = nullptr; int lut_state = 0;
    int calib_blocks = -1;
    double calib_err = 0.0;
    int auto_resolved = -1;
    char* blob = nullptr;
    size_t blob_bytes = 0;
    std::vector<moe::ConvLayer> convs;
    std::map<std::string, int> conv_index;
    std::map<std::string, size_t> small;
    std::map<std::string, float> scalars;
    int max_groups = 256;
    std::vector<std::string> prof_keys;
    bool debug = false;
    moe::StreamSet set;
    moe::PipeSet pipe[2];
    int pipe_next = 0;
    bool pipe_prev_valid = false;
    hipStream_t pipe_last_stream = nullptr;
    moe::NetRuntime rt;

    const moe::Param* get(const std::string& n) const
    {
        auto it = index.find(n);
        return it == index.end() ? nullptr : &params[it->second];
    }
    void add(const std::string& n, std::vector<int64_t> shape)
    {
        index[n] = (int)params.size();
        moe::Param p; p.name = n; p.shape = std::move(shape);
        params.push_back(std::move(p));
    }
};

namespace moe {

struct FwdIO {
    const void* x = nullptr; int x_dtype = MOE_F32; long long sB = 0, sH = 0, sW = 0; const long long* x_off = nullptr;
    void* y = nullptr; int y_dtype = MOE_F32; const long long* y_off = nullptr;
};

struct FwdCtx {
    StreamSet* set = nullptr;
    int groups = 0;
    bool fork = false;
    hipEvent_t gate_event = nullptr;
    float* lut_capture = nullptr;
};
inline FwdCtx own_ctx(const moe_net& n, StreamSet* set) { return FwdCtx{set, n.max_groups, n.opt.branch_streams != 0, nullptr, nullptr}; }

struct ConvExtra {
    const half_t* plane_w = nullptr;
    const half_t* plane_w_lo = nullptr;
    const half_t* tail_w = nullptr;
    float* tplanes = nullptr;
    const float* tail1_w = nullptr;
    float* tail1_out = nullptr;
    bool exact = false;
    float* pool_out = nullptr;
    int pool_slabs = 0;
    bool pool_act = false;
    const float* gate_in = nullptr;
    bool fuse_tail = false, fuse_tail1 = false, pool = false, gate = false;
};
struct ConvDone {
    bool ok = true;
    bool pooled = false;
    bool gated = false;
    int tail1_parts = 0;
    explicit operator bool() const { return ok; }
};
enum class ConvKernel {
    none, direct, conv1x1,
    mfma, sp, rw, ps4_store,
    sp_res_lo,
    mfma_x3,
    x3, q8, sq,
    sp_three, acc32,
};
struct ConvRoute {
    ConvKernel kernel = ConvKernel::none;
    ConvDone done;
    ConvForm form;
    ConvX3Form x3;
};
const char* kernel_name(ConvKernel k);

struct Fwd {
    const moe_net& n;
    const FwdCtx& ctx;
    NetRuntime* rt;
    hipStream_t s;
    int B, h, w;
    Arena ar;
    int groups;
    bool x3, direct;
    bool mixed = false;
    bool y_vec = false;
    float* acc32 = nullptr;
    size_t acc32_elems = 0;
    half_t* side16 = nullptr;
    bool dry() const { return ar.base == nullptr; }
    int rc = 0;
    bool skips_planned_work = false;
    int tail_form = 0;
    FwdIO io;

    Act act(long long pixels, int ch = 64, bool want_lo = false)
    {
        Act a;
        a.hi = (half_t*)ar.take((size_t)pixels * ch * 2 + 2048);
        if (x3 || want_lo) { a.lo = (half_t*)ar.take((size_t)pixels * ch * 2 + 2048); a.has_lo = true; }
        return a;
    }
    template <typename T> T* blob(size_t off) const { return (T*)(n.blob + off); }
    template <typename T> T* small(const std::string& k) const { return (T*)(n.blob + n.small.at(k)); }

    void tap(const std::string& name, const Act& a, int H, int W, int cs, int C)
    {
        if (!n.debug || dry()) return;
        auto& t = rt->taps[name];
        if (t.dev) { (void)hipFree(t.dev); t.dev = nullptr; }
        const size_t nel = (size_t)B * C * H * W;
        if (hipMalloc((void**)&t.dev, nel * 4) != hipSuccess) return;
        t.shape[0] = B; t.shape[1] = C; t.shape[2] = H; t.shape[3] = W;
        launch_nhwc_to_nchw_f32(a.hi, a.lo, t.dev, B, H, W, cs, C, s);
    }

    bool tail_split_for(const std::string& key) const
    {
        const int mode = n.opt.tail_split;
        return mode == 2 || (mode == 1 && key.compare(0, 8, "convt_R1") == 0);
    }

    int prof_begin(const std::string& key, double flops)
    {
        for (size_t i = 0; i < n.prof_keys.size(); ++i) {
            if (key.find(n.prof_keys[i]) == std::string::npos) continue;
            if (rt->prof_used == rt->prof_ev.size()) {
                NetRuntime::ProfRec r;
                if (hipEventCreate(&r.e0) != hipSuccess || hipEventCreate(&r.e1) != hipSuccess) return -1;
                rt->prof_ev.push_back(r);
            }
            NetRuntime::ProfRec& r = rt->prof_ev[rt->prof_used];
            r.key = (int)i; r.flops = flops;
            (void)hipEventRecord(r.e0, s);
            return (int)rt->prof_used++;
        }
        return -1;
    }
    void prof_end(int rec) { if (rec >= 0) (void)hipEventRecord(rt->prof_ev[rec].e1, s); }
    int repeats(const std::string& key) const { return (!n.opt.repeat_key.empty() && key.find(n.opt.repeat_key) != std::string::npos) ? n.opt.repeat_n : 1; }

    bool use_q8() const { return mixed && (n.opt.x3_impl == 2 || (n.opt.x3_impl == 0 && (n.scale > 1 || n.arch == MOE_ARCH_NETDN))); }
    bool q8_capable(const ConvLayer& L) const
    {
        ConvX3Form c;
        c.B = B; c.H = h; c.W = w; c.slope = L.slope; c.in8 = c.out8 = true;
        return n.opt.x3_fuse && n.opt.conv_impl == 2 && L.k == 3 && L.r == 1 && L.nchunks == 1 && L.nseg == 1 && !L.per_plane && L.wq_hi8 && L.w_arsb_lo && !L.has_bias && conv64_q8_applicable(c);
    }

    ConvDone conv(const std::string& key, const Act& in, const Act& out, const Act* res, int H, int W, const ConvExtra& extra = ConvExtra{});
    ConvRoute route(const std::string& key, const Act& in, const Act& out, const Act* res, int H, int W, const ConvExtra& extra = ConvExtra{}) const;
    ConvForm form(const ConvLayer& L, int H, int W) const;
    int launch(const ConvRoute& r, const std::string& key, const Act& in, const Act& out, const Act* res, const ConvExtra& extra);
    void stem(const Act& out, const Act* out2 = nullptr);
    void tail(const Act* r, const Act* u, int H, int W, bool skip);
    void gate();
};

int forward_arsb(const moe_net& n, Fwd& f);
int forward_sedn(const moe_net& n, Fwd& f);
int forward_lite(const moe_net& n, Fwd& f);

int exact_blocks_of(const moe_net& n);
int default_exact_blocks(int arch);
long long sp_bytes_per_pixel(const moe_net& n);
constexpr long long kSpRange = (1ll << 32) - (1ll << 16);
int forward_dev(moe_net& n, const FwdIO& io, int B, int h, int w, hipStream_t s, bool y_off_mult8, const FwdCtx& ctx);
void free_set(StreamSet& set);
void pipe_destroy(moe_net& n);
void free_records(NetRuntime& rt);
int build_device_weights(moe_net& n, int precision);
void drop_lut(moe_net& n);
bool calibratable(const moe_net& n);
int calibrate_blocks(moe_net& n, double target, hipStream_t s);
int calibrate_sedn(moe_net& n, double target, hipStream_t s, bool adopt);

}
```

### moephoto_amd/csrc/plan_run.cpp

```cpp
#include "net.h"

using namespace moe;

static int plan_device_tables(const Plan& p, int device, int C, int64_t sC, int64_t sH, int64_t sW, int si, int scnt,
                              PlanDeviceCache** outp)
{
    if (scnt < 1) { scnt = 1; si = 0; }
    for (auto& up : p.dev) {
        PlanDeviceCache& d = *up;
        if (d.blob && d.device == device && d.C == C && d.sC == sC && d.sH == sH && d.sW == sW && d.shard_index == si && d.shard_count == scnt) {
            *outp = &d;
            return MOE_OK;
        }
    }
    if (p.dev.size() >= 16) {
        if (p.dev.front()->blob) (void)hipFree(p.dev.front()->blob);
        for (auto& e : p.dev.front()->strip_tabs) (void)hipFree(e.second);
        p.dev.erase(p.dev.begin());
    }
    p.dev.push_back(std::make_unique<PlanDeviceCache>());
    PlanDeviceCache& d = *p.dev.back();
    const size_t nt = p.tiles.size();
    std::vector<long long> xo, yo;
    int slot = 0;
    for (const auto& g : p.groups) {
        d.group_first.push_back(slot);
        int cnt = 0;
        for (int k : g.tiles) {
            if (k % scnt != si) continue;
            const TileRect& t = p.tiles[k];
            const long long plane = (long long)(g.th * p.sc) * (g.tw * p.sc);
            for (int c = 0; c < C; ++c) {
                xo.push_back((long long)c * sC + (long long)t.top * sH + (long long)t.left * sW);
                yo.push_back(p.tile_off[k] / p.C * C + (long long)c * plane);
            }
            ++slot; ++cnt;
        }
        d.group_count.push_back(cnt);
    }
    if (xo.empty()) { xo.push_back(0); yo.push_back(0); }
    d.y_mult8 = true;
    for (long long v : yo) d.y_mult8 = d.y_mult8 && (v % 8 == 0);
    std::vector<long long> toff(nt);
    for (size_t k = 0; k < nt; ++k) toff[k] = p.tile_off[k] / p.C * C;
    std::vector<char> host;
    auto put = [&](const void* src, size_t bytes) { const size_t a = (host.size() + 255) & ~(size_t)255; host.resize(a + bytes); memcpy(host.data() + a, src, bytes); return a; };
    const size_t o_x = put(xo.data(), xo.size() * 8), o_y = put(yo.data(), yo.size() * 8), o_t = put(toff.data(), toff.size() * 8);
    const size_t o_rf = put(p.row_first.data(), p.row_first.size() * 4), o_rc = put(p.row_cnt.data(), p.row_cnt.size() * 4);
    const size_t o_cf = put(p.col_first.data(), p.col_first.size() * 4), o_cc = put(p.col_cnt.data(), p.col_cnt.size() * 4);
    const size_t o_rt = put(p.row_tab.data(), p.row_tab.size() * 4), o_ct = put(p.col_tab.data(), p.col_tab.size() * 4);
    const float zero = 0.f;
    const size_t o_rp = put(p.ramp.empty() ? &zero : p.ramp.data(), std::max<size_t>(4, p.ramp.size() * 4));
    HIP_TRY(hipMalloc(&d.blob, host.size()));
    HIP_TRY(hipMemcpy(d.blob, host.data(), host.size(), hipMemcpyHostToDevice));
    char* b = (char*)d.blob;
    d.x_off = (long long*)(b + o_x); d.y_off = (long long*)(b + o_y); d.tile_off = (long long*)(b + o_t);
    d.row_first = (int*)(b + o_rf); d.row_cnt = (int*)(b + o_rc); d.col_first = (int*)(b + o_cf); d.col_cnt = (int*)(b + o_cc);
    d.row_tab = (int*)(b + o_rt); d.col_tab = (int*)(b + o_ct); d.ramp = (float*)(b + o_rp);
    d.device = device; d.C = C; d.sC = sC; d.sH = sH; d.sW = sW; d.shard_index = si; d.shard_count = scnt;
    *outp = &d;
    return MOE_OK;
}

static void fill_stitch(const Plan& p, const PlanDeviceCache& d, StitchArgs& a, const float* tiles, const long long* tile_off, int C, void* out, int out_dtype)
{
    a.tiles = tiles; a.tile_off = tile_off;
    a.row_first = d.row_first; a.row_cnt = d.row_cnt; a.col_first = d.col_first; a.col_cnt = d.col_cnt;
    a.row_tab = d.row_tab; a.col_tab = d.col_tab; a.ramp = d.ramp;
    a.out = out; a.out_dtype = out_dtype; a.C = C; a.out_h = p.out_h; a.out_w = p.out_w; a.step_w = p.aw.step;
    a.y0 = 0; a.rows = p.out_h; a.row_lo = 0;
}

struct moe_plan { Plan p; };

extern "C" {

int moe_plan_create(const int64_t shape[3], double ram, double ram_coef, int pad, int scale, int align, int cropsize, moe_plan** out)
{
    if (!shape || !out) return fail(MOE_EINVAL, "moe_plan_create: NULL argument");
    auto p = std::make_unique<moe_plan>();
    std::string err;
    int rc = build_plan(p->p, shape, ram, ram_coef, pad, scale, align, cropsize, err);
    if (rc) return fail(rc, "%s", err.c_str());
    *out = p.release();
    return MOE_OK;
}

void moe_plan_destroy(moe_plan* p)
{
    if (!p) return;
    for (auto& d : p->p.dev) { if (d->blob) (void)hipFree(d->blob); for (auto& e : d->strip_tabs) (void)hipFree(e.second); }
    for (auto& d : p->p.fdev) if (d->blob) (void)hipFree(d->blob);
    for (auto& c : p->p.custom_off) if (c.dev) (void)hipFree(c.dev);
    if (p->p.pool) (void)hipFree(p->p.pool);
    delete p;
}

int moe_plan_info(const moe_plan* p, int64_t info[12])
{
    if (!p || !info) return fail(MOE_EINVAL, "moe_plan_info: NULL argument");
    const Plan& q = p->p;
    const int64_t v[12] = {(int64_t)q.tiles.size(), q.ah.step, q.aw.step, q.out_h, q.out_w, q.pad_h_to, q.pad_w_to, q.pad_sc,
                           q.tile_h, q.tile_w, q.ah.clip, q.aw.clip};
    memcpy(info, v, sizeof v);
    return MOE_OK;
}

int moe_plan_rows(const moe_plan* p, int32_t* rows)
{
    if (!p || !rows) return fail(MOE_EINVAL, "moe_plan_rows: NULL argument");
    memcpy(rows, p->p.row_tab.data(), p->p.row_tab.size() * 4);
    return MOE_OK;
}

static void axis_seams(const std::vector<int>& tab, int i, int out[4])
{
    const int n = (int)tab.size() / 4;
    const int o = tab[i * 4 + 2], ext = tab[i * 4 + 3];
    std::vector<std::pair<int, int>> iv;
    for (int k = 0; k < n; ++k) {
        const int a = std::max(tab[k * 4 + 0] - o, 0), b = std::min(tab[k * 4 + 1] - o, ext);
        if (b > a) iv.push_back({a, b});
    }
    std::sort(iv.begin(), iv.end());
    std::vector<std::pair<int, int>> m;
    for (auto& v : iv) {
        if (!m.empty() && v.first <= m.back().second) m.back().second = std::max(m.back().second, v.second);
        else m.push_back(v);
    }
    while (m.size() > 2) { m[1].second = m.back().second; m.pop_back(); }
    out[0] = out[1] = out[2] = out[3] = 0;
    if (m.size() >= 1) { out[0] = m[0].first; out[1] = m[0].second; out[2] = out[3] = m[0].second; }
    if (m.size() == 2) { out[2] = m[1].first; out[3] = m[1].second; }
}

int moe_plan_seams(const moe_plan* p, int32_t* seams)
{
    if (!p || !seams) return fail(MOE_EINVAL, "moe_plan_seams: NULL argument");
    const Plan& q = p->p;
    for (int i = 0; i < q.ah.step; ++i)
        for (int j = 0; j < q.aw.step; ++j) {
            int r[4], c[4];
            axis_seams(q.row_tab, i, r);
            axis_seams(q.col_tab, j, c);
            int32_t* o = seams + ((size_t)i * q.aw.step + j) * 8;
            for (int e = 0; e < 4; ++e) { o[e] = r[e]; o[4 + e] = c[e]; }
        }
    return MOE_OK;
}

static_assert(sizeof(moe_wire_rec) == sizeof(WireRec) && sizeof(WireRec) == 64, "moe_wire_rec layout");

int64_t moe_wire_words(const moe_wire_rec* rec)
{
    if (!rec) return -1;
    WireRec r;
    memcpy(&r, rec, sizeof r);
    return wire_rec_words(r);
}

static int wire_call(bool pack, float* tiles, void* wire, const moe_wire_rec* recs_dev, int n, int64_t max_elems, void* stream)
{
    if (n < 0 || (n > 0 && (!tiles || !wire || !recs_dev))) return fail(MOE_EINVAL, "moe_wire_%s: bad argument", pack ? "pack" : "unpack");
    launch_wire(pack, tiles, (unsigned*)wire, (const WireRec*)recs_dev, n, max_elems, (hipStream_t)stream);
    hipError_t e = hipGetLastError();
    if (e != hipSuccess) return fail(MOE_EHIP, "wire kernel launch failed: %s", hipGetErrorString(e));
    return MOE_OK;
}

int moe_wire_pack(const float* tiles_dev, void* wire_dev, const moe_wire_rec* recs_dev, int n, int64_t max_elems, void* stream)
{
    return wire_call(true, (float*)tiles_dev, wire_dev, recs_dev, n, max_elems, stream);
}

int moe_wire_unpack(float* tiles_dev, const void* wire_dev, const moe_wire_rec* recs_dev, int n, int64_t max_elems, void* stream)
{
    return wire_call(false, tiles_dev, (void*)wire_dev, recs_dev, n, max_elems, stream);
// ... 71 lines not shown
    StitchArgs a{};
    fill_stitch(p->p, *d, a, tiles_dev, (const long long*)tile_off_dev, C, out, out_dtype);
    launch_stitch(a, (hipStream_t)stream);
    hipError_t e = hipGetLastError();
    if (e != hipSuccess) return fail(MOE_EHIP, "stitch launch failed: %s", hipGetErrorString(e));
    return MOE_OK;
}

int moe_stitch_band(const moe_plan* p, int device, const float* tiles_dev, const int64_t* tile_off_dev, int C, void* out, int out_dtype,
                    int row0, int row1, int strip, void* stream)
{
    if (!p || !tiles_dev || !tile_off_dev || !out || C < 1) return fail(MOE_EINVAL, "moe_stitch_band: bad argument");
    const Plan& q = p->p;
    const int nrow = q.ah.step;
    if (row0 < 0 || row1 <= row0 || row1 > nrow) return fail(MOE_EINVAL, "moe_stitch_band: tile rows [%d, %d) of %d", row0, row1, nrow);
    HIP_TRY(hipSetDevice(device));
    PlanDeviceCache* d = nullptr;
    int rc = plan_device_tables(q, device, C, 0, 0, 0, 0, 1, &d);
    if (rc) return rc;
    StitchArgs a{};
    fill_stitch(q, *d, a, tiles_dev, (const long long*)tile_off_dev, C, out, out_dtype);
    a.row_lo = row0;
    a.y0 = q.row_tab[row0 * 4 + 1];
    a.rows = (row1 < nrow ? q.row_tab[row1 * 4 + 1] : q.out_h) - a.y0;
    if (strip && row1 < nrow) {
        int* tab = nullptr;
        for (auto& e : d->strip_tabs) if (e.first == row1) tab = e.second;
        if (!tab) {
            std::vector<int> rt(q.row_tab);
            rt[row1 * 4 + 2] = rt[row1 * 4 + 0];
            rt[row1 * 4 + 3] = rt[row1 * 4 + 1] - rt[row1 * 4 + 0];
            HIP_TRY(hipMalloc((void**)&tab, rt.size() * 4));
            HIP_TRY(hipMemcpy(tab, rt.data(), rt.size() * 4, hipMemcpyHostToDevice));
            d->strip_tabs.push_back({row1, tab});
        }
        a.row_tab = tab;
    }
    launch_stitch(a, (hipStream_t)stream);
    hipError_t e = hipGetLastError();
    if (e != hipSuccess) return fail(MOE_EHIP, "stitch launch failed: %s", hipGetErrorString(e));
    return MOE_OK;
}

int moe_blend_tile(const void* r, int64_t r_sC, int64_t r_sH, void* canvas, int64_t c_sC, int64_t c_sH, int dtype, int C,
                   int top_sc, int left_sc, int bsc, int rsc, int topT, int leftT, int pad_sc, const void* ramp, void* stream)
{
    if (!r || !canvas || C < 1) return fail(MOE_EINVAL, "moe_blend_tile: NULL argument");
    if (dtype != MOE_F32 && dtype != MOE_F16) return fail(MOE_EINVAL, "moe_blend_tile: dtype must be MOE_F32 or MOE_F16");
    const int rh = bsc - top_sc, rw = rsc - left_sc;
    if (rh < 1 || rw < 1 || top_sc < 0 || left_sc < 0 || pad_sc < 0) return fail(MOE_EINVAL, "moe_blend_tile: empty or negative window (%d..%d, %d..%d)", top_sc, bsc, left_sc, rsc);
    auto band = [&](int lt, int l, int& first, int& solid) {
        if (lt < 0) lt += l;
        if (lt < 1) { first = solid = 0; return true; }
        first = lt - pad_sc; solid = lt;
        return first >= 0 && lt <= l;
    };
    BlendTileArgs a{};
    if (!band(topT, rh, a.r0, a.lt_h) || !band(leftT, rw, a.c0, a.lt_w))
        return fail(MOE_EINVAL, "moe_blend_tile: blend band outside the window (topT %d, leftT %d, pad_sc %d, window %d x %d)", topT, leftT, pad_sc, rh, rw);
    if ((a.lt_h > a.r0 || a.lt_w > a.c0) && !ramp) return fail(MOE_EINVAL, "moe_blend_tile: ramp is NULL");
    a.r = r; a.canvas = canvas; a.ramp = ramp; a.r_sC = r_sC; a.r_sH = r_sH; a.c_sC = c_sC; a.c_sH = c_sH;
    a.C = C; a.rh = rh; a.rw = rw; a.top_sc = top_sc; a.left_sc = left_sc;
    launch_blend_tile(a, dtype == MOE_F16, (hipStream_t)stream);
    hipError_t e = hipGetLastError();
    if (e != hipSuccess) return fail(MOE_EHIP, "blend launch failed: %s", hipGetErrorString(e));
    return MOE_OK;
}

int moe_run_plan_ex(moe_net* n, const moe_plan* pl, const void* img, int img_dtype, int64_t sC, int64_t sH, int64_t sW,
                    void* out, int out_dtype, int max_tiles, float* pool, int shard_index, int shard_count, int do_stitch, void* stream)
{
    if (!n || !pl || !img || (do_stitch && !out)) return fail(MOE_EINVAL, "moe_run_plan: NULL argument");
    if (!n->finalized) return fail(MOE_ESTATE, "moe_run_plan: net is not finalized");
    const Plan& p = pl->p;
    if (p.sc != n->scale) return fail(MOE_EINVAL, "moe_run_plan: plan scale %d != net scale %d", p.sc, n->scale);
    if (shard_count < 1) { shard_count = 1; shard_index = 0; }
    if (shard_index < 0 || shard_index >= shard_count) return fail(MOE_EINVAL, "moe_run_plan: shard %d of %d", shard_index, shard_count);
    hipStream_t s = (hipStream_t)stream;
    HIP_TRY(hipSetDevice(n->device));
    const int C = p.C;
    PlanDeviceCache* d = nullptr;
    int rc = plan_device_tables(p, n->device, C, sC, sH, sW, shard_index, shard_count, &d);
    if (rc) return rc;
    if (!pool) {
        const size_t pool_need = p.pool_elems_per_plane_set;
        if (pool_need > p.pool_elems) {
            if (p.pool) { HIP_TRY(hipStreamSynchronize(s)); HIP_TRY(hipFree(p.pool)); p.pool = nullptr; p.pool_elems = 0; }
            if (hipMalloc((void**)&p.pool, pool_need * 4) != hipSuccess) { (void)hipGetLastError(); return fail(MOE_ENOMEM, "tile pool of %zu bytes does not fit", pool_need * 4); }
            p.pool_elems = pool_need;
        }
        pool = p.pool;
    }
    if (max_tiles <= 0) {
        max_tiles = n->opt.tiles_per_batch > 0 ? n->opt.tiles_per_batch : 32;
    }
    for (size_t gi = 0; gi < p.groups.size(); ++gi) {
        const auto& g = p.groups[gi];
        const int nt = d->group_count[gi];
        if (nt < 1) continue;
        const long long px = (long long)g.th * g.tw;
        const int per = (int)std::max<long long>(1, std::min<long long>(nt, (long long)max_tiles * 65536 / std::max<long long>(px, 1)));
        for (int t0 = 0; t0 < nt; t0 += per) {
            const int cnt = std::min(per, nt - t0);
            const long long slot = (long long)(d->group_first[gi] + t0) * C;
            rc = forward_dev(*n, FwdIO{img, img_dtype, 0, sH, sW, d->x_off + slot, pool, MOE_F32, d->y_off + slot}, cnt * C, g.th, g.tw, s, d->y_mult8, own_ctx(*n, &n->set));
            if (rc) return rc;
        }
    }
    if (do_stitch) {
        StitchArgs a{};
        fill_stitch(p, *d, a, pool, d->tile_off, C, out, out_dtype);
        launch_stitch(a, s);
        hipError_t e = hipGetLastError();
        if (e != hipSuccess) return fail(MOE_EHIP, "stitch launch failed: %s", hipGetErrorString(e));
    }
    return MOE_OK;
}

int moe_run_plan_tiles(moe_net* n, const moe_plan* pl, const void* imgs, int img_dtype, int64_t frame_stride,
                       int64_t sC, int64_t sH, int64_t sW, int n_frames, float* dst, const int64_t* tile_dst,
                       int max_tiles, void* stream)
{
    if (!n || !pl || !imgs || !dst || !tile_dst || n_frames < 1) return fail(MOE_EINVAL, "moe_run_plan_tiles: bad argument");
    if (!n->finalized) return fail(MOE_ESTATE, "moe_run_plan_tiles: net is not finalized");
    const Plan& p = pl->p;
    if (p.sc != n->scale) return fail(MOE_EINVAL, "moe_run_plan_tiles: plan scale %d != net scale %d", p.sc, n->scale);
    hipStream_t s = (hipStream_t)stream;
    HIP_TRY(hipSetDevice(n->device));
    const int C = p.C;
    const long long nt = (long long)p.tiles.size();
    FramesDeviceCache* d = nullptr;
    for (auto& up : p.fdev) {
        FramesDeviceCache& c = *up;
        if (c.blob && c.device == n->device && c.C == C && c.sC == sC && c.sH == sH && c.sW == sW && c.frame_stride == frame_stride &&
            c.n_frames == n_frames && c.tile_dst.size() == (size_t)(nt * n_frames) &&
            std::equal(c.tile_dst.begin(), c.tile_dst.end(), tile_dst)) { d = &c; break; }
    }
    if (!d) {
        if (p.fdev.size() >= 8) {
            HIP_TRY(hipStreamSynchronize(s));
            if (p.fdev.front()->blob) (void)hipFree(p.fdev.front()->blob);
            p.fdev.erase(p.fdev.begin());
        }
        p.fdev.push_back(std::make_unique<FramesDeviceCache>());
        d = p.fdev.back().get();
        std::vector<long long> xo, yo;
        int slot = 0;
        for (const auto& g : p.groups) {
            d->group_first.push_back(slot);
            int cnt = 0;
            const long long plane = (long long)(g.th * p.sc) * (g.tw * p.sc);
            for (int f = 0; f < n_frames; ++f)
                for (int k : g.tiles) {
                    const long long at = tile_dst[(long long)f * nt + k];
                    if (at < 0) continue;
                    const TileRect& t = p.tiles[k];
                    for (int c = 0; c < C; ++c) {
                        xo.push_back((long long)f * frame_stride + (long long)c * sC + (long long)t.top * sH + (long long)t.left * sW);
                        yo.push_back(at + (long long)c * plane);
                    }
                    ++slot; ++cnt;
                }
            d->group_count.push_back(cnt);
        }
        if (xo.empty()) { xo.push_back(0); yo.push_back(0); }
        d->y_mult8 = true;
        for (long long v : yo) d->y_mult8 = d->y_mult8 && (v % 8 == 0);
        HIP_TRY(hipMalloc(&d->blob, xo.size() * 16));
        d->x_off = (long long*)d->blob; d->y_off = d->x_off + xo.size();
        HIP_TRY(hipMemcpy(d->x_off, xo.data(), xo.size() * 8, hipMemcpyHostToDevice));
        HIP_TRY(hipMemcpy(d->y_off, yo.data(), yo.size() * 8, hipMemcpyHostToDevice));
        d->device = n->device; d->C = C; d->sC = sC; d->sH = sH; d->sW = sW; d->frame_stride = frame_stride;
        d->n_frames = n_frames; d->tile_dst.assign(tile_dst, tile_dst + nt * n_frames);
    }
    if (max_tiles <= 0) {
        max_tiles = n->opt.tiles_per_batch > 0 ? n->opt.tiles_per_batch : 32;
    }
    for (size_t gi = 0; gi < p.groups.size(); ++gi) {
        const auto& g = p.groups[gi];
        const int ntl = d->group_count[gi];
        if (ntl < 1) continue;
        const long long px = (long long)g.th * g.tw;
        const int per = (int)std::max<long long>(1, std::min<long long>(ntl, (long long)max_tiles * 65536 / std::max<long long>(px, 1)));
        for (int t0 = 0; t0 < ntl; t0 += per) {
            const int cnt = std::min(per, ntl - t0);
            const long long slot = (long long)(d->group_first[gi] + t0) * C;
            int rc = forward_dev(*n, FwdIO{imgs, img_dtype, 0, sH, sW, d->x_off + slot, dst, MOE_F32, d->y_off + slot}, cnt * C, g.th, g.tw, s, d->y_mult8, own_ctx(*n, &n->set));
            if (rc) return rc;
        }
    }
    return MOE_OK;
}

int moe_run_plan_frames(moe_net* n, const moe_plan* pl, const void* imgs, int img_dtype, int64_t frame_stride,
                        int64_t sC, int64_t sH, int64_t sW, int n_frames, float* pools, int64_t pool_stride,
                        int owner_index, int owner_count, int max_tiles, void* stream)
{
    if (!n || !pl || !imgs || !pools || n_frames < 1) return fail(MOE_EINVAL, "moe_run_plan_frames: bad argument");
    const Plan& p = pl->p;
    if (owner_count < 1) { owner_count = 1; owner_index = 0; }
    if (owner_index < 0 || owner_index >= owner_count) return fail(MOE_EINVAL, "moe_run_plan_frames: owner %d of %d", owner_index, owner_count);
    if (pool_stride < (int64_t)p.pool_elems_per_plane_set) return fail(MOE_EINVAL, "moe_run_plan_frames: pool stride smaller than one frame's pool");
    const long long nt = (long long)p.tiles.size();
    std::vector<int64_t> at((size_t)(nt * n_frames));
    for (int f = 0; f < n_frames; ++f)
        for (long long k = 0; k < nt; ++k)
            at[(size_t)(f * nt + k)] = ((f * nt + k) % owner_count == owner_index) ? (int64_t)f * pool_stride + p.tile_off[(size_t)k] : -1;
    return moe_run_plan_tiles(n, pl, imgs, img_dtype, frame_stride, sC, sH, sW, n_frames, pools, at.data(), max_tiles, stream);
}

int moe_run_plan(moe_net* n, const moe_plan* pl, const void* img, int img_dtype, int64_t sC, int64_t sH, int64_t sW,
                 void* out, int out_dtype, int max_tiles, void* stream)
{
    return moe_run_plan_ex(n, pl, img, img_dtype, sC, sH, sW, out, out_dtype, max_tiles, nullptr, 0, 1, 1, stream);
}

int moe_to_float(const void* src, int src_dtype, int bits, int H, int W, int C, void* dst, int dst_dtype, int device, void* stream)
{
    if (!src || !dst || H < 1 || W < 1 || C < 1) return fail(MOE_EINVAL, "moe_to_float: bad argument");
    if ((src_dtype != MOE_U8 && src_dtype != MOE_U16) || (dst_dtype != MOE_F32 && dst_dtype != MOE_F16)) return fail(MOE_EINVAL, "moe_to_float: bad dtype");
    HIP_TRY(hipSetDevice(device));
    if (src_dtype == MOE_U8) launch_to_float(src, src_dtype, 255.f, true, H, W, C, dst, dst_dtype, (hipStream_t)stream);
    else launch_to_float(src, src_dtype, 1.f / (float)(1 << bits), false, H, W, C, dst, dst_dtype, (hipStream_t)stream);
    return MOE_OK;
}

int moe_resize(const void* src, void* dst, int dtype, int C, int H, int W, int h, int w, int mode, int device, void* stream)
{
    if (!src || !dst || C < 1 || H < 1 || W < 1 || h < 1 || w < 1) return fail(MOE_EINVAL, "moe_resize: bad argument");
    if (dtype != MOE_F32 && dtype != MOE_F16) return fail(MOE_EINVAL, "moe_resize: dtype must be MOE_F32 or MOE_F16");
    if (mode < MOE_RESIZE_NEAREST || mode > MOE_RESIZE_BICUBIC) return fail(MOE_EINVAL, "moe_resize: unknown mode %d", mode);
    HIP_TRY(hipSetDevice(device));
    launch_resize(src, dst, dtype, C, H, W, h, w, mode, (hipStream_t)stream);
    hipError_t e = hipGetLastError();
    if (e != hipSuccess) return fail(MOE_EHIP, "resize launch failed: %s", hipGetErrorString(e));
    return MOE_OK;
}

int moe_to_output(const void* src, int src_dtype, int H, int W, int C, int bits, void* dst, int dst_dtype, int device, void* stream)
{
    if (!src || !dst || H < 1 || W < 1 || C < 1 || bits < 1 || bits > 16) return fail(MOE_EINVAL, "moe_to_output: bad argument");
    if ((dst_dtype != MOE_U8 && dst_dtype != MOE_U16) || (src_dtype != MOE_F32 && src_dtype != MOE_F16)) return fail(MOE_EINVAL, "moe_to_output: bad dtype");
    if (dst_dtype == MOE_U8 && bits > 8) return fail(MOE_EINVAL, "moe_to_output: %d bits do not fit MOE_U8", bits);
    HIP_TRY(hipSetDevice(device));
    launch_to_output(src, src_dtype, H, W, C, (float)(1 << bits), dst, dst_dtype, (hipStream_t)stream);
    return MOE_OK;
}

}
```

### moephoto_amd/imageProcess.py

```python
import ctypes
import logging
import time
from functools import reduce

import numpy as np
import torch
import torch.nn.functional as F

from . import _lib
from .config import config
from .models import EngineModule
from .weights import load_state_dict_file

log = logging.getLogger('Moe')
modelCache = {}
weightCache = {}
minSize = 28
PLAN_CACHE = 4
identity = lambda x, *_, **__: x
apply = lambda v, f: f(v)
_DT = {torch.float32: _lib.F32, torch.float16: _lib.F16}


def ceilBy(d):
    return lambda x: ((int(x) + d - 1) // d) * d


alignF = {1: identity}
alignF.update((1 << k, ceilBy(1 << k)) for k in (3, 4, 5, 6, 7, 9))


class TilePlan(object):

    def __init__(self, shape, ram, ramCoef, pad, sc, align=8, cropsize=0):
        L = _lib.lib()
        self.shape = tuple(int(v) for v in shape[-3:])
        self._h = ctypes.c_void_p()
        _lib.check(L.moe_plan_create((ctypes.c_int64 * 3)(*self.shape), float(ram), float(ramCoef), int(pad), int(sc),
                                     int(align), int(cropsize), ctypes.byref(self._h)))
        info = (ctypes.c_int64 * 12)()
        _lib.check(L.moe_plan_info(self._h, info))
        (self.n_tiles, self.stepH, self.stepW, self.outH, self.outW, self.padHTo, self.padWTo, self.padSc,
         self.tileH, self.tileW, self.clipH, self.clipW) = [int(v) for v in info]
        t = (ctypes.c_int32 * (8 * self.n_tiles))()
        _lib.check(L.moe_plan_tiles(self._h, t))
        self.tiles = [tuple(t[k * 8:(k + 1) * 8]) for k in range(self.n_tiles)]
        r = (ctypes.c_float * max(1, self.padSc))()
        _lib.check(L.moe_plan_ramp(self._h, r))
        self.ramp = np.array(r[:self.padSc], np.float32)
        rt = (ctypes.c_int32 * (4 * self.stepH))()
        _lib.check(L.moe_plan_rows(self._h, rt))
        self.rows = [tuple(rt[i * 4:(i + 1) * 4]) for i in range(self.stepH)]
        self.sc, self.pad, self.align = int(sc), int(pad), int(align)

    def __del__(self):
        try:
            if self._h.value:
                _lib.lib().moe_plan_destroy(self._h)
                self._h = ctypes.c_void_p()
        except Exception:
            pass

    def pool_elems(self, C):
        return int(_lib.check(_lib.lib().moe_plan_pool_elems(self._h, int(C))))

    def tile_offsets(self, C):
        off = (ctypes.c_int64 * self.n_tiles)()
        _lib.check(_lib.lib().moe_plan_tile_offsets(self._h, int(C), off))
        return list(off)

    def seams(self):
        t = (ctypes.c_int32 * (8 * self.n_tiles))()
        _lib.check(_lib.lib().moe_plan_seams(self._h, t))
        return [tuple(t[k * 8:(k + 1) * 8]) for k in range(self.n_tiles)]

    def padImage(self, x):
        def pad_axis(t, from_end, to):
            n = t.shape[-from_end]
            if not to or to <= n:
                return t
            refl = min(n - 1, to - n)
            if refl > 0:
                p = (0, refl, 0, 0) if from_end == 1 else (0, 0, 0, refl)
                t = F.pad(t.unsqueeze(0), p, mode='reflect').squeeze(0)
            rest = to - n - refl
            if rest > 0:
                t = F.pad(t, (0, rest, 0, 0) if from_end == 1 else (0, 0, 0, rest))
            return t
        x = pad_axis(x, 1, self.padWTo)
        x = pad_axis(x, 2, self.padHTo)
        return x

    def unpad(self, im):
        return im[..., :self.outH, :self.outW]


def getAnchors(s, ns, l, pad, af, sc):
    n = l - 2 * pad
    step = 1 if l >= af(s) else max(2, -(-int(ns) // n))
    start = [k * n + pad for k in range(step)]
    start[0] = 0
    end = [a + l for a in start]
    endSc = [e * sc for e in end]
    if step > 1:
        start[-1] = s - af(s - end[-2] + pad)
        end[-1] = s
        clip = int((end[-2] - s) * sc)
    else:
        end[-1] = af(s)
        clip = 0
    endSc[-1] = s * sc
    return start, end, clip, step, [int(e) for e in endSc]


def prepare(shape, ram, opt, pad, sc, align=8, cropsize=0):
    plan = TilePlan(shape, ram, opt.ramCoef, pad, sc, align, cropsize)

    def iterClip():
        for t in plan.tiles:
            yield t
    iterClip.plan = plan
    b = torch.from_numpy(plan.ramp.copy()).view(1, -1)
    return iterClip, plan.padImage, plan.unpad, (*shape[:-2], plan.outH, plan.outW), b


class Option(object):
    _DEFAULTS = dict(ramCoef=1e-3, count=0, padding=1, cropsize=0, align=8, fixChannel=1, scale=1, ensemble=0, strength=1.0,
                     outShape=None, oShape=None, iterClip=None, modelCached=None)

    def __init__(self, path=''):
        for name, value in self._DEFAULTS.items():
            setattr(self, name, value)
        self.model = path
        self.prepare = identity
        self.squeeze = lambda t: t.squeeze(0)
        self.unsqueeze = lambda t: t.unsqueeze(0)
        self._plans = {}

    def __call__(self, x, *args, **kwargs):
        result = self.modelCached(x, *args, **kwargs)
        return result[-1] if isinstance(result, list) else result


def getStateDict(path):
    if path not in weightCache:
        sd = load_state_dict_file(path)
        weightCache[path] = type(sd)((k, torch.from_numpy(v)) for k, v in sd.items())
    return weightCache[path]


def castModel(model):
    return model.to(dtype=config.dtype(), device=config.device())
# ... 324 lines not shown
```

Before: 88.55 MP/s.

## Defer ps4 tail-add into stitch, reading pixel-shuffle planes directly

When the ps4 upsampling tail is used, each launch set's pixel-shuffle planes and aprons are kept in a per-plan persistent buffer, and the separate tail-add kernel that wrote the fp32 tile pool is skipped. A new stitch kernel variant sums the planes and apron corrections on the fly while blending tiles into the output. This removes one full write and read of the upscaled tile pool. The cost is a larger persistent plane buffer, extra per-pixel indexing in stitch, and more scattered reads at seams. It is on by default when the call conditions hold.

Result: slower. 87.42 MP/s (-1.3%).

```diff
diff --git a/include/moephoto_amd.h b/include/moephoto_amd.h
--- a/include/moephoto_amd.h
+++ b/include/moephoto_amd.h
@@ -108,6 +108,9 @@
                     void* out, int out_dtype, int max_tiles_per_batch, float* pool, int shard_index, int shard_count,
                     int do_stitch, void* stream);
 
+int moe_plan_set_defer_tailadd(moe_plan* plan, int enable);
+int moe_run_plan_defers(const moe_net* net, const moe_plan* plan, int max_tiles_per_batch);
+
 int moe_run_plan_frames(moe_net* net, const moe_plan* plan, const void* imgs, int img_dtype, int64_t frame_stride,
                         int64_t sC, int64_t sH, int64_t sW, int n_frames, float* pools, int64_t pool_stride,
                         int owner_index, int owner_count, int max_tiles_per_batch, void* stream);
diff --git a/moephoto_amd/_lib.py b/moephoto_amd/_lib.py
--- a/moephoto_amd/_lib.py
+++ b/moephoto_amd/_lib.py
@@ -78,6 +78,8 @@
         'moe_stitch': (c_int, [c_vp, c_int, c_vp, c_vp, c_int, c_vp, c_int, c_vp]),
         'moe_run_plan': (c_int, [c_vp, c_vp, c_vp, c_int, c_i64, c_i64, c_i64, c_vp, c_int, c_int, c_vp]),
         'moe_run_plan_ex': (c_int, [c_vp, c_vp, c_vp, c_int, c_i64, c_i64, c_i64, c_vp, c_int, c_int, c_vp, c_int, c_int, c_int, c_vp]),
+        'moe_plan_set_defer_tailadd': (c_int, [c_vp, c_int]),
+        'moe_run_plan_defers': (c_int, [c_vp, c_vp, c_int]),
         'moe_run_plan_frames': (c_int, [c_vp, c_vp, c_vp, c_int, c_i64, c_i64, c_i64, c_i64, c_int, c_vp, c_i64, c_int, c_int, c_int, c_vp]),
         'moe_run_plan_tiles': (c_int, [c_vp, c_vp, c_vp, c_int, c_i64, c_i64, c_i64, c_i64, c_int, c_vp, P(c_i64), c_int, c_vp]),
         'moe_to_float': (c_int, [c_vp, c_int, c_int, c_int, c_int, c_int, c_vp, c_int, c_int, c_vp]),
@@ -97,7 +99,7 @@
            'moe_net_num_params', 'moe_net_param_info', 'moe_net_set_param', 'moe_net_finalize', 'moe_net_resolved_precision', 'moe_net_calibrate', 'moe_net_exact_blocks', 'moe_net_workspace_bytes',
            'moe_net_max_tile_pixels', 'moe_net_forward', 'moe_net_forward_ex', 'moe_net_set_profile', 'moe_net_get_profile', 'moe_net_get_profile_at', 'moe_net_set_exact_blocks', 'moe_net_set_debug', 'moe_net_set_option', 'moe_device_info', 'moe_blend_tile', 'moe_stitch_dev', 'moe_stitch_band', 'moe_net_debug_tap', 'moe_plan_create', 'moe_plan_destroy', 'moe_plan_info',
            'moe_plan_tiles', 'moe_plan_ramp', 'moe_plan_rows', 'moe_plan_seams', 'moe_wire_words', 'moe_wire_pack', 'moe_wire_unpack', 'moe_plan_pool_elems', 'moe_plan_tile_offsets', 'moe_stitch', 'moe_run_plan',
-           'moe_run_plan_ex', 'moe_run_plan_frames', 'moe_run_plan_tiles', 'moe_to_float', 'moe_to_output', 'moe_resize']
+           'moe_run_plan_ex', 'moe_plan_set_defer_tailadd', 'moe_run_plan_defers', 'moe_run_plan_frames', 'moe_run_plan_tiles', 'moe_to_float', 'moe_to_output', 'moe_resize']
 
 
 def check(rc):
diff --git a/moephoto_amd/build.py b/moephoto_amd/build.py
--- a/moephoto_amd/build.py
+++ b/moephoto_amd/build.py
@@ -7,7 +7,7 @@
 CSRC = os.path.join(HERE, 'csrc')
 SOURCES = ['conv_mfma.hip', 'conv3x3_sp.hip', 'conv3x3_rw.hip', 'conv3x3_ps4.hip', 'conv3x3_ps9.hip', 'arsb32c.hip', 'conv64_x3.hip', 'conv64_q8.hip', 'conv64_sq.hip', 'arsb_sq.hip', 'conv64_s.hip', 'conv1x1.hip', 'conv1x1_f2.hip', 'misc_kernels.hip', 'blend.hip',
            'errors.cpp', 'options.cpp', 'weights.cpp', 'forward.cpp', 'forward_arsb.cpp', 'forward_sedn.cpp', 'forward_lite.cpp', 'calibrate.cpp', 'plan_run.cpp', 'planner.cpp']
-HEADERS = ['common.h', 'engine.h', 'net.h', 'rowtile.h', os.path.join('..', '..', 'include', 'moephoto_amd.h')]
+HEADERS = ['common.h', 'engine.h', 'net.h', 'plane_sets.h', 'rowtile.h', 'tailadd.h', os.path.join('..', '..', 'include', 'moephoto_amd.h')]
 LIB = os.path.join(HERE, 'libmoephoto_amd.so')
 ARCH = 'gfx950'
 EXTRA_FLAGS = {'blend.hip': ['-ffp-contract=off'],
diff --git a/moephoto_amd/csrc/common.h b/moephoto_amd/csrc/common.h
--- a/moephoto_amd/csrc/common.h
+++ b/moephoto_amd/csrc/common.h
@@ -363,8 +363,15 @@
 };
 void launch_frm_pre(const FrmPreArgs& a, hipStream_t s);
 
+struct PlaneSet {
+    const float* p0; const float* p1;
+    const float* a0; const float* a1;
+    int B, H, W, px;
+};
+
 struct StitchArgs {
     const float* tiles; const long long* tile_off;
+    const PlaneSet* sets; const int* tile_set;
     const int* row_first; const int* row_cnt;
     const int* col_first; const int* col_cnt;
     const int* row_tab; const int* col_tab;
diff --git a/moephoto_amd/csrc/conv3x3_ps4.hip b/moephoto_amd/csrc/conv3x3_ps4.hip
--- a/moephoto_amd/csrc/conv3x3_ps4.hip
+++ b/moephoto_amd/csrc/conv3x3_ps4.hip
@@ -1,5 +1,6 @@
 #include "common.h"
 #include "rowtile.h"
+#include "tailadd.h"
 #include "../../include/moephoto_amd.h"
 #include <algorithm>
 #include <type_traits>
@@ -503,30 +504,8 @@
     const int xq = (int)(idx % nq);
     const int Y = (int)((idx / nq) % a.H), b = (int)(idx / ((long long)nq * a.H));
     const int X0 = xq * 8;
-    const long long po = ((long long)b * a.H + Y) * a.W + X0;
     float v[8];
-    {
-        const float4 r0 = *(const float4*)(a.p0 + po), r1 = *(const float4*)(a.p0 + po + 4);
-        v[0] = r0.x; v[1] = r0.y; v[2] = r0.z; v[3] = r0.w; v[4] = r1.x; v[5] = r1.y; v[6] = r1.z; v[7] = r1.w;
-        if (a.p1) {
-            const float4 u0 = *(const float4*)(a.p1 + po), u1 = *(const float4*)(a.p1 + po + 4);
-            v[0] += u0.x; v[1] += u0.y; v[2] += u0.z; v[3] += u0.w; v[4] += u1.x; v[5] += u1.y; v[6] += u1.z; v[7] += u1.w;
-        }
-    }
-    const int c = X0 >> 6, in = X0 & 63;
-    const long long as = (long long)a.B * a.px * a.H;
-    if (in == 0 && c >= 1) {
-        const long long o = ((long long)b * a.px + (c - 1)) * a.H + Y;
-        float t = a.a0[o];
-        if (a.a1) t += a.a1[o];
-        v[0] += t;
-    }
-    if (in == 56 && c + 1 < a.px) {
-        const long long o = as + ((long long)b * a.px + (c + 1)) * a.H + Y;
-        float t = a.a0[o];
-        if (a.a1) t += a.a1[o];
-        v[7] += t;
-    }
+    tailadd_vals<8>(a.p0, a.p1, a.a0, a.a1, a.B, a.H, a.W, a.px, b, Y, X0, v);
     const long long yo = (a.y_off ? a.y_off[b] : (long long)b * a.H * a.W) + (long long)Y * a.W + X0;
     if (a.y_dtype == MOE_F16) {
         if (VEC) {
diff --git a/moephoto_amd/csrc/engine.h b/moephoto_amd/csrc/engine.h
--- a/moephoto_amd/csrc/engine.h
+++ b/moephoto_amd/csrc/engine.h
@@ -49,6 +49,13 @@
 
 struct CustomOffsets { int device; std::vector<long long> host; long long* dev; };
 
+struct DeferCache {
+    char* planes = nullptr; size_t planes_bytes = 0;
+    void* tab = nullptr; size_t tab_bytes = 0;
+    std::vector<char> tab_host;
+    int device = -1;
+};
+
 struct TileGroup { int th, tw; std::vector<int> tiles; int first_slot; };
 
 struct Plan {
@@ -66,6 +73,8 @@
     mutable std::vector<CustomOffsets> custom_off;
     mutable float* pool = nullptr;
     mutable size_t pool_elems = 0;
+    mutable DeferCache defer;
+    int defer_tailadd = 1;
 };
 int build_plan(Plan& p, const int64_t shape[3], double ram, double ram_coef, int pad, int sc, int align, int cropsize,
                std::string& err);
diff --git a/moephoto_amd/csrc/forward.cpp b/moephoto_amd/csrc/forward.cpp
--- a/moephoto_amd/csrc/forward.cpp
+++ b/moephoto_amd/csrc/forward.cpp
@@ -349,6 +349,13 @@
     return f.ar.off + 4096;
 }
 
+bool forward_tail_is_ps4(const moe_net& n, const FwdCtx& ctx, int B, int h, int w)
+{
+    if (!n.finalized || B < 1 || h < 1 || w < 1 || (long long)B > kSpRange / (sp_bytes_per_pixel(n) * (long long)h * w)) return false;
+    Fwd f = make_fwd(n, ctx, nullptr, nullptr, B, h, w, Arena{});
+    return run_forward(n, f, FwdIO{}) == MOE_OK && f.tail_ps4;
+}
+
 static bool plan_matches(const Fwd& f, size_t planned)
 {
     if (f.ar.overflow) return false;
@@ -402,6 +409,7 @@
                     h, w, kSpRange / sp_bytes_per_pixel(n));
     if (n.arch == MOE_ARCH_LITE && io.x_dtype == MOE_F16 && n.lut_state == 0 && n.opt.lite_lut) build_lite_lut(n, s, ctx);
     if (B <= bmax) return forward_dev_chunk(n, io, B, h, w, s, y_off_mult8, ctx);
+    if (ctx.planes) return fail(MOE_EINVAL, "internal error: planes deferred for %d planes of %dx%d, which run as several launch sets", B, h, w);
     const size_t xe = io.x_dtype == MOE_F32 ? 4 : 2, ye = io.y_dtype == MOE_F32 ? 4 : 2;
     const long long yplane = (long long)h * n.scale * w * n.scale;
     for (int b0 = 0; b0 < B; b0 += (int)bmax) {
diff --git a/moephoto_amd/csrc/forward_arsb.cpp b/moephoto_amd/csrc/forward_arsb.cpp
--- a/moephoto_amd/csrc/forward_arsb.cpp
+++ b/moephoto_amd/csrc/forward_arsb.cpp
@@ -79,13 +79,21 @@
         ps4 = ok && n.opt.up_impl == 1 && ps4_ok && (2 * wl) % 8 == 0;
         ps9 = fuse && n.opt.up_impl == 1 && n.r == 3 && f.groups >= 3 && ps9_ok;
     }
+    f.tail_ps4 = ps4;
 }
 
 template <typename Args, typename Launch>
 int ArsbRun::ps_stage(int br, const std::string& key, const Act& cur, size_t plane_bytes, size_t apron_bytes, const char* name, Launch launch)
 {
-    ps_plane[br] = (float*)f.ar.take(plane_bytes + 4096);
-    ps_apron[br] = (float*)f.ar.take(apron_bytes + 4096);
+    if (const TailPlanes* d = f.ctx.planes) {
+        if (plane_bytes + 4096 > d->plane_bytes || apron_bytes + 4096 > d->apron_bytes)
+            return fail(MOE_EINVAL, "internal error: layer %s needs %zu + %zu bytes of deferred planes, the caller's slices hold %zu + %zu", key.c_str(), plane_bytes + 4096, apron_bytes + 4096,
+                        d->plane_bytes, d->apron_bytes);
+        ps_plane[br] = d->plane[br]; ps_apron[br] = d->apron[br];
+    } else {
+        ps_plane[br] = (float*)f.ar.take(plane_bytes + 4096);
+        ps_apron[br] = (float*)f.ar.take(apron_bytes + 4096);
+    }
     if (!f.dry()) {
         const ConvLayer& L = n.convs[n.conv_index.at(key)];
         Args q{};
@@ -235,6 +243,7 @@
 
 int ArsbRun::branch_sum()
 {
+    if (ps4 && f.ctx.planes) return MOE_OK;
     if (ps4) { tail_add<TailAddArgs>(launch_tailadd); return MOE_OK; }
     if (ps9) { tail_add<TailAdd3Args>(launch_tailadd3); return MOE_OK; }
     if (fuse) {
@@ -272,6 +281,7 @@
     f.stem(A);
     f.tap("stem", A, h, w, 64, n.C);
     plan_tail_form();
+    if (f.ctx.planes && !ps4) return fail(MOE_EINVAL, "internal error: planes deferred for a launch set (%d planes of %dx%d) that does not take the ps4 form", B, h, w);
     const bool forked = sr && f.ctx.fork && !n.debug && !f.direct && !f.x3 && n.opt.conv_impl == 2 && (long long)B * h * w <= 4ll * 65536;
     struct ForkGuard {
         StreamSet* set; hipStream_t s; bool armed = false;
diff --git a/moephoto_amd/csrc/misc_kernels.hip b/moephoto_amd/csrc/misc_kernels.hip
--- a/moephoto_amd/csrc/misc_kernels.hip
+++ b/moephoto_amd/csrc/misc_kernels.hip
@@ -1,4 +1,5 @@
 #include "common.h"
+#include "tailadd.h"
 #include <algorithm>
 #include <cstdlib>
 #include <cstring>
@@ -986,7 +987,48 @@
     }
 }
 
-__device__ __forceinline__ float stitch_pixel(const StitchArgs& a, int X, int Y, int c)
+struct PoolSrc {
+    const StitchArgs& a;
+    __device__ __forceinline__ float at(int k, int c, int eh, int ew, int y, int x) const { return a.tiles[a.tile_off[k] + ((long long)c * eh + y) * ew + x]; }
+    __device__ __forceinline__ void oct(int k, int c, int eh, int ew, int y, int x, float (&q)[8]) const
+    {
+        const long long o = a.tile_off[k] + ((long long)c * eh + y) * ew + x;
+        if ((o & 3) == 0) {
+            const float4 q0 = *(const float4*)(a.tiles + o), q1 = *(const float4*)(a.tiles + o + 4);
+            q[0] = q0.x; q[1] = q0.y; q[2] = q0.z; q[3] = q0.w; q[4] = q1.x; q[5] = q1.y; q[6] = q1.z; q[7] = q1.w;
+        } else {
+#pragma unroll
+            for (int e = 0; e < 8; ++e) q[e] = a.tiles[o + e];
+        }
+    }
+};
+struct PlaneSrc {
+    const StitchArgs& a;
+    __device__ __forceinline__ float at(int k, int c, int, int, int y, int x) const
+    {
+        const PlaneSet& s = a.sets[a.tile_set[2 * k]];
+        float v[1];
+        tailadd_vals<1>(s.p0, s.p1, s.a0, s.a1, s.B, s.H, s.W, s.px, a.tile_set[2 * k + 1] + c, y, x, v);
+        return v[0];
+    }
+    __device__ __forceinline__ void oct(int k, int c, int, int, int y, int x, float (&q)[8]) const
+    {
+        const PlaneSet& s = a.sets[a.tile_set[2 * k]];
+        const int b = a.tile_set[2 * k + 1] + c;
+        if ((x & 7) == 0) tailadd_vals<8>(s.p0, s.p1, s.a0, s.a1, s.B, s.H, s.W, s.px, b, y, x, q);
+        else {
+#pragma unroll
+            for (int e = 0; e < 8; ++e) {
+                float v[1];
+                tailadd_vals<1>(s.p0, s.p1, s.a0, s.a1, s.B, s.H, s.W, s.px, b, y, x + e, v);
+                q[e] = v[0];
+            }
+        }
+    }
+};
+
+template <typename Src>
+__device__ __forceinline__ float stitch_pixel(const StitchArgs& a, const Src& src, int X, int Y, int c)
 {
     const int i0 = a.row_first[Y], ni = a.row_cnt[Y];
     const int j0 = a.col_first[X], nj = a.col_cnt[X];
@@ -995,7 +1037,7 @@
         const int fy = a.row_tab[i * 4 + 0], sy = a.row_tab[i * 4 + 1], oy = a.row_tab[i * 4 + 2], eh = a.row_tab[i * 4 + 3];
         for (int j = j0; j < j0 + nj; ++j) {
             const int fx = a.col_tab[j * 4 + 0], sx = a.col_tab[j * 4 + 1], ox = a.col_tab[j * 4 + 2], ew = a.col_tab[j * 4 + 3];
-            const float r = a.tiles[a.tile_off[i * a.step_w + j] + ((long long)c * eh + (Y - oy)) * ew + (X - ox)];
+            const float r = src.at(i * a.step_w + j, c, eh, ew, Y - oy, X - ox);
             float v1 = r;
             if (Y < sy) v1 = cur + a.ramp[Y - fy] * (r - cur);
             float v = v1;
@@ -1005,6 +1047,7 @@
     }
     return cur;
 }
+__device__ __forceinline__ float stitch_pixel(const StitchArgs& a, int X, int Y, int c) { return stitch_pixel(a, PoolSrc{a}, X, Y, c); }
 
 __global__ __launch_bounds__(256) void stitch_kernel(StitchArgs a)
 {
@@ -1050,8 +1093,8 @@
     }
 }
 
-template <int R>
-__global__ __launch_bounds__(256) void stitch8r_kernel(StitchArgs a)
+template <int R, typename Src>
+__device__ __forceinline__ void stitch8r_body(const StitchArgs& a, const Src& src)
 {
     __shared__ int s_col[64 * 4];
     __shared__ int s_seam[256];
@@ -1078,15 +1121,8 @@
                 float cur[8] = {0.f, 0.f, 0.f, 0.f, 0.f, 0.f, 0.f, 0.f};
                 for (int i = max(i0, a.row_lo); i < i0 + ni; ++i) {
                     const int fy = a.row_tab[i * 4 + 0], sy = a.row_tab[i * 4 + 1], oy = a.row_tab[i * 4 + 2], eh = a.row_tab[i * 4 + 3];
-                    const long long o = a.tile_off[i * nsw + j0] + ((long long)c * eh + (Y - oy)) * ew + (X0 - ox);
                     float q[8];
-                    if ((o & 3) == 0) {
-                        const float4 q0 = *(const float4*)(a.tiles + o), q1 = *(const float4*)(a.tiles + o + 4);
-                        q[0] = q0.x; q[1] = q0.y; q[2] = q0.z; q[3] = q0.w; q[4] = q1.x; q[5] = q1.y; q[6] = q1.z; q[7] = q1.w;
-                    } else {
-#pragma unroll
-                        for (int e = 0; e < 8; ++e) q[e] = a.tiles[o + e];
-                    }
+                    src.oct(i * nsw + j0, c, eh, ew, Y - oy, X0 - ox, q);
                     if (Y < sy) {
                         const float wgt = a.ramp[Y - fy];
 #pragma unroll
@@ -1122,12 +1158,18 @@
         const int r = rem >> 3, e = rem & 7;
         const int X = (blockIdx.x * 256 + s_seam[gidx]) * 8 + e, Y = Y0 + r;
         if (Y >= yend) continue;
-        const float cur = stitch_pixel(a, X, Y, c);
+        const float cur = stitch_pixel(a, src, X, Y, c);
         const long long o = ((long long)c * a.rows + (Y - a.y0)) * a.out_w + X;
         if (a.out_dtype == MOE_F16) ((half_t*)a.out)[o] = (half_t)cur;
         else ((float*)a.out)[o] = cur;
     }
 }
+
+template <int R>
+__global__ __launch_bounds__(256) void stitch8r_kernel(StitchArgs a) { stitch8r_body<R>(a, PoolSrc{a}); }
+
+template <int R>
+__global__ __launch_bounds__(256) void stitch8p_kernel(StitchArgs a) { stitch8r_body<R>(a, PlaneSrc{a}); }
 
 template <typename TS, typename TD>
 __global__ void to_float_kernel(const TS* src, TD* dst, int H, int W, int C, float d, bool divide)
@@ -1299,6 +1341,10 @@
 void launch_stitch(const StitchArgs& a, hipStream_t s)
 {
     if (a.rows <= 0) return;
+    if (a.sets) {
+        hipLaunchKernelGGL(stitch8p_kernel<4>, dim3((a.out_w / 8 + 255) / 256, (a.rows + 3) / 4, a.C), dim3(256), 0, s, a);
+        return;
+    }
     if (a.out_w % 8 == 0 && a.step_w <= 64 && ((uintptr_t)a.out & 15) == 0) hipLaunchKernelGGL(stitch8r_kernel<4>, dim3((a.out_w / 8 + 255) / 256, (a.rows + 3) / 4, a.C), dim3(256), 0, s, a);
     else if (a.out_w % 4 == 0 && ((uintptr_t)a.out & 15) == 0) hipLaunchKernelGGL(stitch4_kernel, dim3((a.out_w / 4 + 255) / 256, a.rows, a.C), dim3(256), 0, s, a);
     else hipLaunchKernelGGL(stitch_kernel, dim3((a.out_w + 255) / 256, a.rows, a.C), dim3(256), 0, s, a);
diff --git a/moephoto_amd/csrc/net.h b/moephoto_amd/csrc/net.h
--- a/moephoto_amd/csrc/net.h
+++ b/moephoto_amd/csrc/net.h
@@ -170,12 +170,15 @@
     void* y = nullptr; int y_dtype = MOE_F32; const long long* y_off = nullptr;
 };
 
+struct TailPlanes { float* plane[2]; float* apron[2]; size_t plane_bytes, apron_bytes; };
+
 struct FwdCtx {
     StreamSet* set = nullptr;
     int groups = 0;
     bool fork = false;
     hipEvent_t gate_event = nullptr;
     float* lut_capture = nullptr;
+    const TailPlanes* planes = nullptr;
 };
 inline FwdCtx own_ctx(const moe_net& n, StreamSet* set) { return FwdCtx{set, n.max_groups, n.opt.branch_streams != 0, nullptr, nullptr}; }
 
@@ -234,6 +237,7 @@
     int rc = 0;
     bool skips_planned_work = false;
     int tail_form = 0;
+    bool tail_ps4 = false;
     FwdIO io;
 
     Act act(long long pixels, int ch = 64, bool want_lo = false)
@@ -308,6 +312,7 @@
 long long sp_bytes_per_pixel(const moe_net& n);
 constexpr long long kSpRange = (1ll << 32) - (1ll << 16);
 int forward_dev(moe_net& n, const FwdIO& io, int B, int h, int w, hipStream_t s, bool y_off_mult8, const FwdCtx& ctx);
+bool forward_tail_is_ps4(const moe_net& n, const FwdCtx& ctx, int B, int h, int w);
 void free_set(StreamSet& set);
 void pipe_destroy(moe_net& n);
 void free_records(NetRuntime& rt);
diff --git a/moephoto_amd/csrc/plan_run.cpp b/moephoto_amd/csrc/plan_run.cpp
--- a/moephoto_amd/csrc/plan_run.cpp
+++ b/moephoto_amd/csrc/plan_run.cpp
@@ -1,4 +1,5 @@
 #include "net.h"
+#include "plane_sets.h"
 
 using namespace moe;
 
@@ -73,6 +74,73 @@
 
 struct moe_plan { Plan p; };
 
+static std::vector<GroupTiles> group_tiles(const Plan& p, int si, int scnt, std::vector<std::vector<int>>& store)
+{
+    store.assign(p.groups.size(), {});
+    std::vector<GroupTiles> g;
+    for (size_t gi = 0; gi < p.groups.size(); ++gi) {
+        for (int k : p.groups[gi].tiles) if (k % scnt == si) store[gi].push_back(k);
+        g.push_back(GroupTiles{p.groups[gi].th, p.groups[gi].tw, store[gi].data(), (int)store[gi].size()});
+    }
+    return g;
+}
+
+static int default_max_tiles(const moe_net& n, int max_tiles)
+{
+    if (max_tiles > 0) return max_tiles;
+    return n.opt.tiles_per_batch > 0 ? n.opt.tiles_per_batch : 32;
+}
+
+static bool defer_applies(const moe_net& n, const Plan& p, const std::vector<LaunchSet>& sets, bool own_pool, int do_stitch, int shard_count, const void* out)
+{
+    if (!defer_call_ok(p.defer_tailadd != 0, own_pool, do_stitch, shard_count, p.out_w, p.aw.step, (uintptr_t)out)) return false;
+    if (!n.finalized || n.r != 2 || !(n.arch == MOE_ARCH_NET2X || n.arch == MOE_ARCH_NET4X) || sets.empty()) return false;
+    const FwdCtx ctx = own_ctx(n, nullptr);
+    for (const LaunchSet& L : sets)
+        if (!forward_tail_is_ps4(n, ctx, L.cnt * p.C, L.th, L.tw)) return false;
+    return true;
+}
+
+static int defer_prepare(const moe_net& n, const Plan& p, const PlaneLayout& lay, hipStream_t s)
+{
+    DeferCache& d = p.defer;
+    if (d.device != n.device && d.device >= 0) {
+        HIP_TRY(hipStreamSynchronize(s));
+        if (d.planes) (void)hipFree(d.planes);
+        if (d.tab) (void)hipFree(d.tab);
+        d = DeferCache{};
+    }
+    d.device = n.device;
+    if (lay.bytes > d.planes_bytes) {
+        if (d.planes) { HIP_TRY(hipStreamSynchronize(s)); HIP_TRY(hipFree(d.planes)); d.planes = nullptr; d.planes_bytes = 0; }
+        if (hipMalloc((void**)&d.planes, lay.bytes) != hipSuccess) { (void)hipGetLastError(); return fail(MOE_ENOMEM, "branch-plane buffer of %zu bytes does not fit", lay.bytes); }
+        d.planes_bytes = lay.bytes;
+    }
+    std::vector<PlaneSet> sets(lay.sets.size());
+    for (size_t i = 0; i < sets.size(); ++i) {
+        const PlaneSlice& q = lay.sets[i];
+        sets[i] = PlaneSet{(const float*)(d.planes + q.plane[0]), (const float*)(d.planes + q.plane[1]), (const float*)(d.planes + q.apron[0]), (const float*)(d.planes + q.apron[1]),
+                           q.B, q.H, q.W, q.px};
+    }
+    const size_t sb = sets.size() * sizeof(PlaneSet), tb = lay.tile_set.size() * sizeof(int);
+    std::vector<char> host(sb + tb);
+    memcpy(host.data(), sets.data(), sb);
+    memcpy(host.data() + sb, lay.tile_set.data(), tb);
+    if (host != d.tab_host) {
+        HIP_TRY(hipStreamSynchronize(s));
+        if (host.size() > d.tab_bytes) {
+            if (d.tab) { HIP_TRY(hipFree(d.tab)); d.tab = nullptr; d.tab_bytes = 0; }
+            d.tab_host.clear();
+            HIP_TRY(hipMalloc(&d.tab, host.size()));
+            d.tab_bytes = host.size();
+        }
+        d.tab_host.clear();
+        HIP_TRY(hipMemcpy(d.tab, host.data(), host.size(), hipMemcpyHostToDevice));
+        d.tab_host = host;
+    }
+    return MOE_OK;
+}
+
 extern "C" {
 
 int moe_plan_create(const int64_t shape[3], double ram, double ram_coef, int pad, int scale, int align, int cropsize, moe_plan** out)
@@ -93,6 +161,8 @@
     for (auto& d : p->p.fdev) if (d->blob) (void)hipFree(d->blob);
     for (auto& c : p->p.custom_off) if (c.dev) (void)hipFree(c.dev);
     if (p->p.pool) (void)hipFree(p->p.pool);
+    if (p->p.defer.planes) (void)hipFree(p->p.defer.planes);
+    if (p->p.defer.tab) (void)hipFree(p->p.defer.tab);
     delete p;
 }
 
@@ -330,7 +400,16 @@
     PlanDeviceCache* d = nullptr;
     int rc = plan_device_tables(p, n->device, C, sC, sH, sW, shard_index, shard_count, &d);
     if (rc) return rc;
-    if (!pool) {
+    max_tiles = default_max_tiles(*n, max_tiles);
+    std::vector<std::vector<int>> store;
+    const std::vector<GroupTiles> groups = group_tiles(p, shard_index, shard_count, store);
+    const std::vector<LaunchSet> sets = launch_sets(groups, max_tiles);
+    PlaneLayout lay;
+    const bool defer = defer_applies(*n, p, sets, pool == nullptr, do_stitch, shard_count, out) &&
+                       plane_layout(groups, sets, (int)p.tiles.size(), C, n->stages, n->r, ps4_plane_bytes, ps4_apron_bytes, lay);
+    if (defer) {
+        if ((rc = defer_prepare(*n, p, lay, s))) return rc;
+    } else if (!pool) {
         const size_t pool_need = p.pool_elems_per_plane_set;
         if (pool_need > p.pool_elems) {
             if (p.pool) { HIP_TRY(hipStreamSynchronize(s)); HIP_TRY(hipFree(p.pool)); p.pool = nullptr; p.pool_elems = 0; }
@@ -339,25 +418,24 @@
         }
         pool = p.pool;
     }
-    if (max_tiles <= 0) {
-        max_tiles = n->opt.tiles_per_batch > 0 ? n->opt.tiles_per_batch : 32;
-    }
-    for (size_t gi = 0; gi < p.groups.size(); ++gi) {
-        const auto& g = p.groups[gi];
-        const int nt = d->group_count[gi];
-        if (nt < 1) continue;
-        const long long px = (long long)g.th * g.tw;
-        const int per = (int)std::max<long long>(1, std::min<long long>(nt, (long long)max_tiles * 65536 / std::max<long long>(px, 1)));
-        for (int t0 = 0; t0 < nt; t0 += per) {
-            const int cnt = std::min(per, nt - t0);
-            const long long slot = (long long)(d->group_first[gi] + t0) * C;
-            rc = forward_dev(*n, FwdIO{img, img_dtype, 0, sH, sW, d->x_off + slot, pool, MOE_F32, d->y_off + slot}, cnt * C, g.th, g.tw, s, d->y_mult8, own_ctx(*n, &n->set));
-            if (rc) return rc;
-        }
+    for (size_t si = 0; si < sets.size(); ++si) {
+        const LaunchSet& L = sets[si];
+        const long long slot = L.slot * C;
+        FwdCtx ctx = own_ctx(*n, &n->set);
+        TailPlanes tp{};
+        if (defer) {
+            const PlaneSlice& q = lay.sets[si];
+            char* b = p.defer.planes;
+            tp = TailPlanes{{(float*)(b + q.plane[0]), (float*)(b + q.plane[1])}, {(float*)(b + q.apron[0]), (float*)(b + q.apron[1])}, q.plane_bytes, q.apron_bytes};
+            ctx.planes = &tp;
+        }
+        rc = forward_dev(*n, FwdIO{img, img_dtype, 0, sH, sW, d->x_off + slot, pool, MOE_F32, d->y_off + slot}, L.cnt * C, L.th, L.tw, s, d->y_mult8, ctx);
+        if (rc) return rc;
     }
     if (do_stitch) {
         StitchArgs a{};
         fill_stitch(p, *d, a, pool, d->tile_off, C, out, out_dtype);
+        if (defer) { a.tiles = nullptr; a.sets = (const PlaneSet*)p.defer.tab; a.tile_set = (const int*)((const char*)p.defer.tab + lay.sets.size() * sizeof(PlaneSet)); }
         launch_stitch(a, s);
         hipError_t e = hipGetLastError();
         if (e != hipSuccess) return fail(MOE_EHIP, "stitch launch failed: %s", hipGetErrorString(e));
@@ -463,6 +541,25 @@
     return moe_run_plan_ex(n, pl, img, img_dtype, sC, sH, sW, out, out_dtype, max_tiles, nullptr, 0, 1, 1, stream);
 }
 
+int moe_plan_set_defer_tailadd(moe_plan* p, int enable)
+{
+    if (!p) return fail(MOE_EINVAL, "moe_plan_set_defer_tailadd: NULL plan");
+    p->p.defer_tailadd = enable != 0;
+    return MOE_OK;
+}
+
+int moe_run_plan_defers(const moe_net* n, const moe_plan* pl, int max_tiles)
+{
+    if (!n || !pl) return fail(MOE_EINVAL, "moe_run_plan_defers: NULL argument");
+    const Plan& p = pl->p;
+    if (p.sc != n->scale) return 0;
+    std::vector<std::vector<int>> store;
+    const std::vector<GroupTiles> groups = group_tiles(p, 0, 1, store);
+    const std::vector<LaunchSet> sets = launch_sets(groups, default_max_tiles(*n, max_tiles));
+    PlaneLayout lay;
+    return defer_applies(*n, p, sets, true, 1, 1, nullptr) && plane_layout(groups, sets, (int)p.tiles.size(), p.C, n->stages, n->r, ps4_plane_bytes, ps4_apron_bytes, lay) ? 1 : 0;
+}
+
 int moe_to_float(const void* src, int src_dtype, int bits, int H, int W, int C, void* dst, int dst_dtype, int device, void* stream)
 {
     if (!src || !dst || H < 1 || W < 1 || C < 1) return fail(MOE_EINVAL, "moe_to_float: bad argument");
diff --git a/moephoto_amd/csrc/plane_sets.h b/moephoto_amd/csrc/plane_sets.h
--- /dev/null
+++ b/moephoto_amd/csrc/plane_sets.h
@@ -0,0 +1,71 @@
+#pragma once
+#include <algorithm>
+#include <cstddef>
+#include <cstdint>
+#include <vector>
+
+namespace moe {
+
+struct GroupTiles { int th, tw; const int* tiles; int count; };
+struct LaunchSet { int group, t0, cnt, th, tw; long long slot; };
+
+inline std::vector<LaunchSet> launch_sets(const std::vector<GroupTiles>& groups, int max_tiles)
+{
+    std::vector<LaunchSet> out;
+    long long slot = 0;
+    for (size_t gi = 0; gi < groups.size(); ++gi) {
+        const GroupTiles& g = groups[gi];
+        const int nt = g.count;
+        const long long px = (long long)g.th * g.tw;
+        const int per = (int)std::max<long long>(1, std::min<long long>(nt, (long long)max_tiles * 65536 / std::max<long long>(px, 1)));
+        for (int t0 = 0; t0 < nt; t0 += per) out.push_back(LaunchSet{(int)gi, t0, std::min(per, nt - t0), g.th, g.tw, slot + t0});
+        slot += nt;
+    }
+    return out;
+}
+
+inline bool defer_call_ok(bool enabled, bool own_pool, int do_stitch, int shard_count, int out_w, int step_w, uintptr_t out)
+{
+    return enabled && own_pool && do_stitch != 0 && shard_count == 1 && out_w > 0 && out_w % 8 == 0 && step_w <= 64 && (out & 15) == 0;
+}
+
+struct PlaneSlice { size_t plane[2], apron[2]; size_t plane_bytes, apron_bytes; int B, H, W, px; };
+struct PlaneLayout {
+    std::vector<PlaneSlice> sets;
+    std::vector<int> tile_set;
+    size_t bytes = 0;
+};
+typedef size_t (*PlaneBytesFn)(int B, int H, int W);
+
+inline bool plane_layout(const std::vector<GroupTiles>& groups, const std::vector<LaunchSet>& sets, int n_tiles, int C, int stages, int r,
+                         PlaneBytesFn plane_fn, PlaneBytesFn apron_fn, PlaneLayout& out)
+{
+    out = PlaneLayout{};
+    if (n_tiles < 1 || C < 1 || stages < 1 || r < 2) return false;
+    out.tile_set.assign((size_t)n_tiles * 2, -1);
+    auto take = [&out](size_t bytes) { const size_t a = (out.bytes + 255) & ~(size_t)255; out.bytes = a + bytes; return a; };
+    for (size_t si = 0; si < sets.size(); ++si) {
+        const LaunchSet& L = sets[si];
+        if (L.group < 0 || (size_t)L.group >= groups.size() || L.cnt < 1 || L.t0 < 0 || L.t0 + L.cnt > groups[(size_t)L.group].count) return false;
+        long long hl = L.th, wl = L.tw;
+        for (int st = 0; st + 1 < stages; ++st) { hl *= r; wl *= r; }
+        const long long B = (long long)L.cnt * C;
+        if (hl < 1 || wl < 1 || hl * r > INT32_MAX || wl * r > INT32_MAX || B > INT32_MAX) return false;
+        PlaneSlice s{};
+        s.B = (int)B; s.H = (int)(hl * r); s.W = (int)(wl * r); s.px = (int)((wl + 31) / 32);
+        s.plane_bytes = plane_fn((int)B, (int)hl, (int)wl) + 4096;
+        s.apron_bytes = apron_fn((int)B, (int)hl, (int)wl) + 4096;
+        for (int br = 0; br < 2; ++br) { s.plane[br] = take(s.plane_bytes); s.apron[br] = take(s.apron_bytes); }
+        out.sets.push_back(s);
+        for (int t = 0; t < L.cnt; ++t) {
+            const int k = groups[(size_t)L.group].tiles[L.t0 + t];
+            if (k < 0 || k >= n_tiles || out.tile_set[(size_t)k * 2] != -1) return false;
+            out.tile_set[(size_t)k * 2] = (int)si;
+            out.tile_set[(size_t)k * 2 + 1] = t * C;
+        }
+    }
+    for (int k = 0; k < n_tiles; ++k) if (out.tile_set[(size_t)k * 2] < 0) return false;
+    return true;
+}
+
+}
diff --git a/moephoto_amd/csrc/tailadd.h b/moephoto_amd/csrc/tailadd.h
--- /dev/null
+++ b/moephoto_amd/csrc/tailadd.h
@@ -0,0 +1,35 @@
+#pragma once
+#include "common.h"
+
+template <int N>
+__device__ __forceinline__ void tailadd_vals(const float* p0, const float* p1, const float* a0, const float* a1,
+                                             int B, int H, int W, int px, int b, int Y, int X0, float (&v)[N])
+{
+    static_assert(N == 8 || N == 1, "an octet or one pixel");
+    const long long po = ((long long)b * H + Y) * W + X0;
+    if constexpr (N == 8) {
+        const float4 r0 = *(const float4*)(p0 + po), r1 = *(const float4*)(p0 + po + 4);
+        v[0] = r0.x; v[1] = r0.y; v[2] = r0.z; v[3] = r0.w; v[4] = r1.x; v[5] = r1.y; v[6] = r1.z; v[7] = r1.w;
+        if (p1) {
+            const float4 u0 = *(const float4*)(p1 + po), u1 = *(const float4*)(p1 + po + 4);
+            v[0] += u0.x; v[1] += u0.y; v[2] += u0.z; v[3] += u0.w; v[4] += u1.x; v[5] += u1.y; v[6] += u1.z; v[7] += u1.w;
+        }
+    } else {
+        v[0] = p0[po];
+        if (p1) v[0] += p1[po];
+    }
+    const int c = X0 >> 6, in = X0 & 63;
+    const long long as = (long long)B * px * H;
+    if (in == 0 && c >= 1) {
+        const long long o = ((long long)b * px + (c - 1)) * H + Y;
+        float t = a0[o];
+        if (a1) t += a1[o];
+        v[0] += t;
+    }
+    if (in == 64 - N && c + 1 < px) {
+        const long long o = as + ((long long)b * px + (c + 1)) * H + Y;
+        float t = a0[o];
+        if (a1) t += a1[o];
+        v[N - 1] += t;
+    }
+}
diff --git a/moephoto_amd/imageProcess.py b/moephoto_amd/imageProcess.py
--- a/moephoto_amd/imageProcess.py
+++ b/moephoto_amd/imageProcess.py
@@ -68,6 +68,12 @@
         off = (ctypes.c_int64 * self.n_tiles)()
         _lib.check(_lib.lib().moe_plan_tile_offsets(self._h, int(C), off))
         return list(off)
+
+    def set_defer_tailadd(self, on):
+        _lib.check(_lib.lib().moe_plan_set_defer_tailadd(self._h, int(bool(on))))
+
+    def defers_tailadd(self, model, max_tiles=0):
+        return bool(_lib.check(_lib.lib().moe_run_plan_defers(model._h, self._h, int(max_tiles))))
 
     def seams(self):
         t = (ctypes.c_int32 * (8 * self.n_tiles))()
```
